# griffithlab/regtools

Hardware: AMD Instinct MI355X
Metric: alignments/sec + junctions/sec, junctions extract, 1/2/4/8 MI355X (higher is better)
Workload: dtype u8/u32 integer; 1 GPU; configs[1]: synthetic 50000000-read 101 bp BAM per GPU, ~15% reads with one N-op, junctions extract -s XS; reads_per_gpu=50000000, seed=1, bgzf_members=169426, compressed_bytes_per_gpu=533101619, inflated_bytes_per_gpu=11060000978

## Files before the change

regtools_amd/csrc/api_internal.h:

```cpp
#pragma once
#include "../../include/regtools_amd.h"

#include <hip/hip_runtime.h>
#include <stdarg.h>
#include <stdio.h>
#include <stdlib.h>
#include <string.h>

#include <algorithm>
#include <atomic>
#include <condition_variable>
#include <charconv>
#include <chrono>
#include <map>
#include <memory>
#include <mutex>
#include <string>
#include <thread>
#include <unordered_map>
#include <vector>

#include "cse_host.h"
#include "host_io.h"
#include "worker_pool.h"
// ... 78 lines not shown
        k.v.erase(k.v.begin() + (long)best);
        return base;
    }
    static void unmap_range(void *base, const std::vector<size_t> &lens, size_t reserved, int dev) {
        static const bool trace = getenv("REGTOOLS_AMD_TRACE") != nullptr;
        size_t at = 0;
        for (size_t n : lens) {
            const hipError_t e = hipMemUnmap((uint8_t *)base + at, n);
            if (e != hipSuccess && trace) fprintf(stderr, "[rgx trace] hipMemUnmap of %zu bytes at +%zu: %s\n", n, at, hipGetErrorString(e));
            if (e != hipSuccess) (void)hipGetLastError();
            at += n;
        }
        KeptRanges &k = kept_ranges();
        std::lock_guard<std::mutex> lock(k.mu);
        k.v.push_back(KeptRange{base, reserved, dev});
    }
    hipError_t map_pieces(size_t bytes, void **out) {
        int dev = 0;
        hipError_t e = hipGetDevice(&dev);
        if (e != hipSuccess) return e;
        hipMemAllocationProp prop = {}; prop.type = hipMemAllocationTypePinned; prop.location.type = hipMemLocationTypeDevice; prop.location.id = dev;
        size_t gran = 0;
        if (hipMemGetAllocationGranularity(&gran, &prop, hipMemAllocationGranularityRecommended) != hipSuccess || !gran) { (void)hipGetLastError();
            gran = (size_t)2 << 20; }
        const size_t total = (bytes + gran - 1) / gran * gran, each = std::max(gran, piece / gran * gran);
        size_t reserved = total;
        void *base = take_range(dev, total, &reserved);
        if (!base) { reserved = total; if ((e = hipMemAddressReserve(&base, total, 0, nullptr, 0)) != hipSuccess) return e; }
        std::vector<size_t> lens;
        size_t done = 0;
        while (done < total) {
            const size_t n = std::min(each, total - done);
            hipMemGenericAllocationHandle_t h;
            if ((e = hipMemCreate(&h, n, &prop, 0)) != hipSuccess) break;
            e = hipMemMap((uint8_t *)base + done, n, 0, h, 0);
            (void)hipMemRelease(h);
            if (e != hipSuccess) break;
            lens.push_back(n);
            done += n;
        }
        if (e == hipSuccess) {
            hipMemAccessDesc ad = {}; ad.location.type = hipMemLocationTypeDevice; ad.location.id = dev; ad.flags = hipMemAccessFlagsProtReadWrite;
            e = hipMemSetAccess(base, total, &ad, 1);
        }
        if (e != hipSuccess) { unmap_range(base, lens, reserved, dev); return e; }
        *out = base; mapped = reserved; range_dev = dev; piece_len.swap(lens);
        return hipSuccess;
    }
    hipError_t ensure(size_t bytes) {
        if (bytes <= cap) return hipSuccess;
        static const bool trace = getenv("REGTOOLS_AMD_TRACE") != nullptr;
        const auto t0 = std::chrono::steady_clock::now();
        release();
        static const bool no_slack = [] { const char *e = getenv("REGTOOLS_AMD_ONE_SHOT"); return e && strcmp(e, "0") != 0; }();
        size_t want = bytes + (no_slack ? 0 : bytes / 8) + 256;
        void *raw = nullptr;
        hipError_t e = hipErrorNotSupported;
        if (piece && want + kFront >= piece) { e = map_pieces(want + kFront, &raw); if (e != hipSuccess) { (void)hipGetLastError(); raw = nullptr;
            mapped = 0; piece_len.clear(); } }
        if (e != hipSuccess) e = hipMalloc(&raw, want + kFront);
        if (e == hipSuccess) { p = (uint8_t *)raw + kFront; cap = want; }
        if (trace) {
            static std::mutex mu; std::lock_guard<std::mutex> lock(mu);
            g_alloc_stats.ms += std::chrono::duration<double, std::milli>(std::chrono::steady_clock::now() - t0).count(); ++g_alloc_stats.calls;
                g_alloc_stats.bytes += want;
        }
        return e;
    }
    void release() {
        if (p && mapped) { (void)hipDeviceSynchronize();
                           unmap_range((uint8_t *)p - kFront, piece_len, mapped, range_dev); }
        else if (p) (void)hipFree((uint8_t *)p - kFront);
        p = nullptr; cap = 0; mapped = 0; piece_len.clear();
    }
    template <class T> T *as() const { return (T *)p; }
    explicit operator Carve() const { return Carve(p, cap); }
};

enum class Buf {
    arena, bad_members, bam, barcode_text, barcodes, cand, cse_assoc, cse_events_all, cse_junction_items, cse_junctions, cse_pairs, cse_variant_hits,
    cse_variants, cse_windows, discover, events, fasta, fasta_tab, gate_done, gate_flags, gtf_tables, hdr_arena, inflate_scratch, members, merge, odd_aux,
    partials, probe_sizes, probe_slots, rank, row_map, rows_out, rows_packed, scalars, seg, seg_chunks, seg_cp, soa, sort, stage, table_dev, tmp, unique,
    count
};

struct RadixSort {
    uint32_t *perm[2], *tmp; uint32_t n; hipStream_t st; uint32_t *key[2] = {nullptr, nullptr};
    int cur = -1;
    const uint32_t *in() const { return cur < 0 ? nullptr : perm[cur]; }
    void passes(const uint32_t *word, uint32_t nbits, int kc) {
        for (uint32_t sh = 0; sh < nbits; sh += 8) {
            const uint32_t bits = std::min<uint32_t>(8, nbits - sh); const int nxt = cur < 0 ? 0 : cur ^ 1;
            if (kc < 0) launch_radix_pass(word, sh, bits, in(), perm[nxt], n, tmp, st);
            else { launch_radix_pass_keyed(word, key[kc], sh, bits, in(), perm[nxt], n, tmp, st); word = key[kc]; kc ^= 1; }
            cur = nxt;
        }
    }
    void by(const uint32_t *word, uint32_t nbits) { passes(word, nbits, -1); }
    void by_keyed(const uint32_t *word, uint32_t nbits) {
        if (cur < 0) return passes(word, nbits, 0);
        launch_gather_u32(n, word, perm[cur], key[0], st);
        passes(key[0], nbits, 1);
    }
    template <class G> void by_gathered(G gather, uint32_t nbits) { gather(in(), key[0]); passes(key[0], nbits, 1); }
    const uint32_t *sorted() const { return perm[cur]; }
    uint32_t *spare() const { return perm[cur ^ 1]; }
    void reset() { cur = -1; }
};

constexpr uint32_t kCcBatch = 4;
struct EdgeList { const uint32_t *a, *b; uint32_t n; };
int components_run(uint32_t n_vertices, const EdgeList *lists, int n_lists, uint32_t *parent, uint32_t *d_flags, hipStream_t st, uint32_t *n_rounds,
                   char *err, size_t errlen);

constexpr int kSideStreams = 2;
struct OverlapKnobs { size_t min_bytes = (size_t)8 << 20; unsigned chunks = 16; uint32_t early_min = 4096; bool early_small = false; };
inline const OverlapKnobs &overlap_knobs() {
    static const OverlapKnobs k = [] {
        OverlapKnobs v;
        if (const char *e = getenv("REGTOOLS_AMD_OVERLAP")) {
            long long a = -1, b = -1, c2 = -1;
            const int n = sscanf(e, "%lld,%lld,%lld", &a, &b, &c2);
            if (n >= 1 && a >= 0) v.min_bytes = (size_t)a;
            if (n >= 2 && b >= 2) v.chunks = (unsigned)std::min<long long>(b, 64);
            if (n >= 3 && c2 >= 1) { v.early_min = (uint32_t)c2; v.early_small = true; }
        }
        return v;
    }();
    return k;
}
struct Turn {
    std::mutex mu; std::condition_variable cv; uint64_t next = 0, serving = 0;
    uint64_t width = 1;
};
struct LinkTurn { Turn wire, chip; };
struct TurnHold {
    Turn *t = nullptr; std::atomic<bool> held{false};
    void take(Turn *x) {
        if (!x || held.load()) return;
        std::unique_lock<std::mutex> lk(x->mu);
        const uint64_t mine = x->next++;
        x->cv.wait(lk, [&] { return mine < x->serving + x->width; });
        t = x; held.store(true);
    }
    void give() { if (held.exchange(false)) { { std::lock_guard<std::mutex> lk(t->mu); ++t->serving; } t->cv.notify_all(); } }
};

struct rgx_ctx {
    int device = 0;
    LinkTurn *link = nullptr;
    TurnHold wire_hold, chip_hold;
    hipStream_t stream = nullptr;
    hipStream_t copy_stream = nullptr, side[kSideStreams] = {};
    bool gate_distrust = false, early_distrust = false;
    bool walk_strict = false;
    bool one_shot = false;
    std::vector<hipEvent_t> chunk_ev;
    uint32_t gate_epoch = 0;
    hipEvent_t ev_ready = nullptr, ev_side[kSideStreams] = {}, ev_packed = nullptr;
    hipEvent_t ev[8] = {};
    uint64_t arena_calibrated_bytes = 0;
    DevBuf *arena_retired = nullptr;
    hipEvent_t ev_trial[2] = {};
    float arena_trial_ms[8] = {}; int arena_trials = 0;
    hipEvent_t ev_launch[2] = {}; bool launch_timed = false;
    DevBuf bufs[(size_t)Buf::count];
    void *pinned = nullptr; size_t pinned_cap = 0;
    std::vector<Member> hm_scratch;
    void *pinned_members = nullptr; size_t pinned_members_cap = 0;
    void *pinned_rows = nullptr; size_t pinned_rows_cap = 0;
    uint64_t last_rows = 0, last_records = 0, last_events = 0, last_bytes = 0; bool last_rows_valid = false;
    struct KPend { hipEvent_t a, b; int slot; };
    std::vector<KPend> kpend; std::vector<hipEvent_t> kfree; double kms[3] = {0, 0, 0};
    uint64_t tables_made = 0;
    std::vector<uint32_t> rank_stage;
    std::string fasta_path;
    rgx::Fasta *fasta = nullptr;
    rgx::Fasta *host_fasta = nullptr; std::string host_fasta_path; uint64_t host_fasta_key[4] = {0, 0, 0, 0};
    DevBuf &buf(Buf b) { return bufs[(size_t)b]; }
};


rgx::Fasta *host_fasta(rgx_ctx *c, const char *path);
void ktime_begin(rgx_ctx *c, int slot);
void ktime_end(rgx_ctx *c);
void ktime_collect(rgx_ctx *c);
hipError_t ensure_upload_streams(rgx_ctx *c);
rgx_junction_table *table_alloc(const BamHeader &h, uint64_t n, bool zero = true, bool pinned = false);
void host_sort_rows(rgx_junction_table *t);
void format_bed12_rows(const rgx_junction_table *t, int only_anchored, uint64_t r0, uint64_t r1, std::string &out);
void *block_take(size_t need, size_t &cap, bool pinned);
void block_give(void *p, size_t cap, bool pinned);
struct TableBox { rgx_junction_table t; void *block; size_t block_cap; bool pinned; };
struct CachedBlock { void *p; size_t cap; bool pinned; };
struct SharedMembers { const std::vector<Member> *members; uint64_t total_inflated; };

struct Prep {
    BamHeader hdr;
    const uint8_t *arena = nullptr;
    ReadSoA soa{};
    EventSoA ev{};
    uint32_t n_rec = 0, n_events = 0, n_range = 0;
    uint64_t n_iterated = 0, total = 0;
    uint32_t framing_sweeps = 0;
    bool stream_ended = false;
    double t_begin = 0;
    struct OddAux { int32_t tid, pos, end; };
    std::vector<OddAux> odd_aux;
    const uint8_t *d_file = nullptr;
};

int prepare_events(rgx_ctx *c, const uint8_t *d_bam_in, const uint8_t *h_bam, size_t bam_len, const uint8_t *bai, size_t bai_len,
                          const rgx_extract_params *p, bool want_read_span, Prep &P, char *err, size_t errlen, const uint32_t *d_true_sizes = nullptr,
                          bool allow_overlap = true, bool region_to_file_end = false, const SharedMembers *shared = nullptr);

constexpr int kGoOn = -1;

struct EventsRun {
    rgx_ctx *c; const uint8_t *d_bam_in; const uint8_t *h_bam; size_t bam_len; const uint8_t *bai; size_t bai_len;
    const rgx_extract_params *p; bool want_read_span; Prep &P; char *err; size_t errlen; const uint32_t *d_true_sizes;
    bool allow_overlap, region_to_file_end; const SharedMembers *shared;
    hipStream_t st = nullptr, copy_q = nullptr;
    double t_begin = 0, t_last = 0; bool trace = false;
    void mark(const char *what) { if (trace) { double t = now_ms(); fprintf(stderr, "[rgx trace] %-28s +%8.3f ms  (at %8.3f)%s\n", what, t - t_last,
        t - t_begin, c->link ? (" clock " + std::to_string(fmod(t, 1e5))).c_str() : ""); t_last = t; } }
    BaiInfo bi; bool bai_ok = false;
    std::vector<uint8_t> index_image;
    std::thread bai_thread;
    const uint8_t *d_bam = nullptr;
    struct Upload {
        std::thread th; std::atomic<uint32_t> recorded{0}; std::atomic<int> err{0};
        std::vector<size_t> end;
        size_t lo = 0, hi = 0, hdr_hi = 0;
        hipStream_t copy_stream = nullptr;
        ~Upload() { if (th.joinable()) th.join(); if (copy_stream) (void)hipStreamSynchronize(copy_stream); }
    } up;
    bool overlap = false, gated = false;
    size_t gate_chunk = 0;
    uint64_t hm_total = 0;
    Scalars *d_sc = nullptr, *h_sc = nullptr;
    template <class T> hipError_t fetch(T &host_member) { return fetch_scalar(d_sc, h_sc, host_member, st); }
    hipError_t complete_upload() {
        if (!h_bam || !(up.lo || (up.hi && up.hi < bam_len))) return hipSuccess;
        if (up.th.joinable()) up.th.join();
        hipError_t e = hipStreamSynchronize(copy_q);
        uint8_t *dst = c->buf(Buf::bam).as<uint8_t>();
        if (e == hipSuccess && up.lo > up.hdr_hi) e = hipMemcpy(dst + up.hdr_hi, h_bam + up.hdr_hi, up.lo - up.hdr_hi, hipMemcpyHostToDevice);
        if (e == hipSuccess && up.hi < bam_len) e = hipMemcpy(dst + up.hi, h_bam + up.hi, bam_len - up.hi, hipMemcpyHostToDevice);
        up.lo = 0; up.hi = bam_len; up.hdr_hi = 0;
        return e;
    }
    uint32_t n_cand = 0;
    uint64_t *cand = nullptr;
    uint32_t *nx[2] = {nullptr, nullptr}, *c_isize = nullptr, *c_reach = nullptr, *c_rank = nullptr, *c_isz2 = nullptr, *c_tmp = nullptr;
    Member *d_members = nullptr; hipMemcpyKind from_members = hipMemcpyDeviceToHost;
    void chain(uint64_t root2) {
        launch_member_link(d_bam, bam_len, cand, n_cand, nx[0], c_isize, c_reach, root2, st);
        int cur = 0;
        for (uint32_t span = 1; span < n_cand; span <<= 1) { launch_member_jump(n_cand, nx[cur], nx[cur ^ 1], c_reach, st); cur ^= 1; }
        launch_member_jump(n_cand, nx[cur], nx[cur ^ 1], c_reach, st);
        launch_scan_u32(c_reach, c_rank, n_cand, &d_sc->n_members, c_tmp, st);
        launch_member_compact(d_bam, bam_len, cand, c_isize, c_reach, c_rank, n_cand, d_members, c_isz2, st);
        if (d_true_sizes) launch_member_fix(d_members, c_isz2, n_cand, &d_sc->n_members, d_true_sizes, st);
        launch_member_upos(d_members, c_isz2, &d_sc->n_members, &d_sc->total_inflated, st);
    }
    bool whole = false, seek = false, chunked = false, geom_chunked_hint = false, empty_stream = false;
    uint64_t seek_voff = 0, cut_lo = 0, cut_hi = UINT64_MAX, total_all = 0, q_upos[3] = {0, 0, 0};
    std::vector<VChunk> chunks;
    uint32_t n_members_all = 0, first_member = 0, stop = 0;
    uint32_t m_lo = 0, m_hi = 0, n_range = 0;
    uint64_t upos_lo = 0, total = 0;
    uint8_t *d_bad = nullptr;
    hipError_t member_at(uint32_t k, Member &m) {
        if (from_members == hipMemcpyHostToHost) { memcpy(&m, d_members + k, sizeof m); return hipSuccess; }
        hipError_t e = hipMemcpyAsync(&m, d_members + k, sizeof m, from_members, st);
        return e == hipSuccess ? hipStreamSynchronize(st) : e;
    }
    hipError_t upos_of(uint32_t k, uint64_t &out_v) {
        if (k >= n_members_all) { out_v = total_all; return hipSuccess; }
        Member m;
        hipError_t e = member_at(k, m);
        out_v = m.upos;
        return e;
    }
    struct EarlyPart { uint32_t members, waves; uint64_t upos; };
    std::vector<EarlyPart> early_parts;
    bool split_B = false; hipEvent_t split_ev = nullptr;
    hipError_t join_B() {
        if (!split_B) return hipSuccess;
        split_B = false;
        return hipStreamWaitEvent(st, split_ev, 0);
    }
    bool spec = false; uint32_t mean_rec = 0;
    BamHeader hdr; int32_t n_ref = 0;
    uint64_t lim = 0, pos0 = 0; bool chain_ended = false;
    ExtractCfg cfg; SegGeom geom; uint32_t seg_bytes = 0;
    std::vector<SegChunk> seg_chunks;
    const uint8_t *arena = nullptr; uint64_t span = 0; uint32_t n_seg = 0, n_rec = 0; bool lite_walk = false;
    uint64_t *seg_start[2] = {nullptr, nullptr}, *seg_exit[2] = {nullptr, nullptr};
    uint32_t *seg_cnt[2] = {nullptr, nullptr}, *seg_base = nullptr;
    uint32_t *seg_iter_e = nullptr, *seg_long_e = nullptr, *seg_long_base_e = nullptr;
    uint16_t *seg_cp = nullptr;
    int cur = 0;
    int frame(uint32_t n_s, uint32_t walk_from, bool &ended) {
        DevBuf &b_tmp = c->buf(Buf::tmp);
        launch_seg_walk(arena, geom, n_s, n_ref, seg_start[cur], seg_exit[cur], seg_cnt[cur], seg_cp, st, walk_from);
        for (int iter = 0;; ++iter) {
            HIP_TRY(hipMemsetAsync(&d_sc->framing, 0xff, sizeof d_sc->framing, st));
            launch_seg_verify(arena, geom, n_s, seg_start[cur], seg_exit[cur], seg_cnt[cur], seg_start[cur ^ 1], seg_exit[cur ^ 1],
                              seg_cnt[cur ^ 1], &d_sc->framing.disagree, seg_cp, st);
            cur ^= 1;
            launch_scan_u32(seg_cnt[cur], seg_base, n_s, &d_sc->n_rec, b_tmp.as<uint32_t>(), st);
            HIP_TRY(fetch(h_sc->n_rec));
            HIP_TRY(fetch(h_sc->framing));
            if (spec && iter == 0) {
                HIP_TRY(fetch(h_sc->inflate));
                HIP_TRY(fetch(h_sc->inflate_early));
            }
            HIP_TRY(hipStreamSynchronize(st));
            if (spec && iter == 0 && (h_sc->inflate.first_bad != 0xffffffffu || h_sc->inflate_early.first_bad != 0xffffffffu)) {
                mark("inflate verdict: not clean, starting over device-resident");
                if (gated) { c->gate_distrust = true; if (trace) fprintf(stderr,
                    "[rgx trace] arrival gate: verdict not clean, this context no longer uses it\n"); }
                HIP_TRY(join_B());
                HIP_TRY(complete_upload());
                HIP_TRY(hipStreamSynchronize(copy_q));
                HIP_TRY(hipStreamSynchronize(st));
                const int rc2 = prepare_events(c, d_bam, nullptr, bam_len, bai, bai_len, p, want_read_span, P, err, errlen, nullptr, false, region_to_file_end);
                P.t_begin = t_begin;
                return rc2;
            }
            ++P.framing_sweeps;
            const Scalars::Framing &fr = h_sc->framing;
            if (fr.chain_end != 0xffffffffu) ended = true;
            if (fr.chain_end != 0xffffffffu && (fr.chain_end < fr.disagree || (fr.disagree == 0xffffffffu && geom.chunks))) {
                launch_seg_truncate(geom, n_s, fr.chain_end, seg_start[cur], seg_exit[cur], seg_cnt[cur], st);
                launch_scan_u32(seg_cnt[cur], seg_base, n_s, &d_sc->n_rec, b_tmp.as<uint32_t>(), st);
                HIP_TRY(fetch(h_sc->n_rec));
                HIP_TRY(hipStreamSynchronize(st));
                break;
            }
            if (fr.disagree == 0xffffffffu) break;
            if (iter > 1 << 20) return fail(err, errlen, RGX_ERR_FORMAT, "regtools_amd: record framing did not converge\n");
        }
        return -1;
    }
    uint32_t sA = 0;
    bool emit_parts_ok = false; uint32_t emit_parts = 0, emit_rows = 0; size_t ev_lay = 0;
    EventSoA ev_e;
    static constexpr size_t kEventRowBytes = 8 * sizeof(uint32_t) + 1;
    EventSoA ev_layout(Carve &w, size_t E) {
        EventSoA v; memset(&v, 0, sizeof v);
        v.tid = w.u32(E); v.start = w.u32(E); v.ilen_cls = w.u32(E); v.ts = w.u32(E); v.te = w.u32(E);
        if (want_read_span) { v.rpos = w.u32(E); v.rend = w.u32(E); }
        if (p->barcodes) v.read = w.u32(E);
        v.strand = w.u8(E);
        return v;
    }
    size_t soa_cap = 0;
    ReadSoA soa;
    uint32_t *ev_base = nullptr, *long_list = nullptr;
    static constexpr size_t kSoaRowBytes = sizeof(uint64_t) + 6 * sizeof(uint32_t) + 1, kSoaRecOffBytes = sizeof(uint64_t);
    int soa_layout(size_t R) {
        DevBuf &b_soa = c->buf(Buf::soa);
        HIP_TRY(b_soa.ensure(R * (kSoaRowBytes + (p->barcodes ? kSoaRecOffBytes : 0)) + 256));
        Carve w(b_soa);
        soa.cig_off = w.u64(R);
        if (p->barcodes) soa.rec_off = w.u64(R);
        soa.tid = w.take<int32_t>(R); soa.pos = w.take<int32_t>(R); soa.flag_nc = w.u32(R);
        soa.n_ev = w.u32(R); ev_base = w.u32(R); long_list = w.u32(R);
        soa.strand = w.u8(R); CARVE_TRY(w, "soa");
        soa_cap = R;
        return kGoOn;
    }
    uint32_t n_events = 0, n_long = 0; uint64_t n_iterated = 0;
    ~EventsRun() {
        if (split_B && split_ev) (void)hipEventSynchronize(split_ev);
        if (bai_thread.joinable()) bai_thread.join();
        if (c->link && !d_bam_in) { c->wire_hold.give(); c->chip_hold.give(); }
    }
    int run();
    int calibrate_arena();
    int stage_upload();
    int stage_members();
    int stage_range_and_inflate();
    int stage_footers_and_header();
    int stage_bounds_and_chains();
    int stage_framing();
    int stage_decode();
    int stage_emit();
};
struct HostRows {
    std::vector<uint32_t> group, start, end, ts, te, count, name_rank, first_seen, last_seen;
    std::vector<uint8_t> strand;
    size_t n = 0;
    const uint32_t *cols = nullptr;
    void append(const HostRows &batch, uint32_t first_window) {
        auto app = [](std::vector<uint32_t> &dst, const std::vector<uint32_t> &src) { dst.insert(dst.end(), src.begin(), src.end()); };
        for (uint32_t g : batch.group) group.push_back(g + first_window);
        app(start, batch.start); app(end, batch.end); app(ts, batch.ts); app(te, batch.te); app(count, batch.count);
        app(name_rank, batch.name_rank); app(first_seen, batch.first_seen); app(last_seen, batch.last_seen);
        strand.insert(strand.end(), batch.strand.begin(), batch.strand.end());
        n += batch.n;
    }
};

struct RowMap { uint32_t *ev_urow = nullptr, *urow_pos = nullptr; };
struct TableSink { const BamHeader *hdr = nullptr; uint32_t min_anchor = 0; rgx_junction_table *table = nullptr; };

int reduce_events(rgx_ctx *c, EventSoA ev, uint32_t n_events, uint32_t group_bits, uint32_t ilen_bits, const uint32_t *rank_of_group_host,
                  uint32_t n_groups, HostRows &R, char *err, size_t errlen, bool view_only = false, RowMap *row_map = nullptr, TableSink *sink = nullptr,
                  bool allow_preagg = true );
int barcode_rows(rgx_ctx *c, const Prep &P, const RowMap &rm, const rgx_extract_params *p, rgx_junction_table *t, char *err, size_t errlen);
void chrom_string_ranks(const BamHeader &hdr, std::vector<uint32_t> &rank_of_tid);
int run_pipeline(rgx_ctx *c, const uint8_t *d_bam_in, const uint8_t *h_bam, size_t bam_len, const uint8_t *bai, size_t bai_len,
                 const rgx_extract_params *p, rgx_junction_table **out, char *err, size_t errlen, const SharedMembers *shared = nullptr);
bool rgx_enable_peer(int a, int b);
int rgx_last_table_pack_async(rgx_ctx *c, const rgx_junction_table *t, void **d_packed, hipEvent_t *done, char *err, size_t errlen);
```

regtools_amd/csrc/api_records.cpp:

```cpp
#include "api_internal.h"

int EventsRun::stage_footers_and_header() {
    DevBuf &b_arena = c->buf(Buf::arena), &b_hdr = c->buf(Buf::hdr_arena), &b_lens = c->buf(Buf::inflate_scratch);
    BamHeader hdr_host;
    mean_rec = 0;
    spec = overlap && !d_true_sizes && !geom_chunked_hint && host_bam_header(h_bam, std::min<size_t>(bam_len, (size_t)8 << 20), hdr_host, nullptr, &mean_rec);
    if (spec) h_sc->inflate = h_sc->inflate_early = InflateStatus{0xffffffffu, 0xffffffffu};
    else {
        HIP_TRY(join_B());
        HIP_TRY(fetch(h_sc->inflate));
        HIP_TRY(fetch(h_sc->inflate_early));
        HIP_TRY(hipStreamSynchronize(st));
    }
    if (!d_true_sizes) {
        auto size_trouble = [](const InflateStatus &s) { return s.first_bad != 0xffffffffu &&
            (s.code == 12u  || s.code == 10u ); };
        bool lies = size_trouble(h_sc->inflate) || size_trouble(h_sc->inflate_early);
        if (!lies && stop < n_members_all) {
            Member ms; uint8_t two[2] = {0, 0};
            HIP_TRY(member_at(stop, ms));
            if (ms.isize == 0 && ms.clen >= 2) {
                if (h_bam && ms.cpos + 2 <= bam_len) memcpy(two, h_bam + ms.cpos, 2);
                else { HIP_TRY(hipMemcpyAsync(two, d_bam + ms.cpos, 2, hipMemcpyDeviceToHost, st)); HIP_TRY(hipStreamSynchronize(st)); }
            }
            lies = !(ms.isize == 0 && two[0] == 3 && two[1] == 0) && ms.isize != 0xffffffffu;
        }
        if (lies) {
            mark("footer mismatch: probing");
            DevBuf &b_slots = c->buf(Buf::probe_slots), &b_sizes = c->buf(Buf::probe_sizes);
            HIP_TRY(b_slots.ensure((size_t)n_members_all * kBgzfMaxBlock + 256));
            HIP_TRY(b_sizes.ensure((size_t)n_members_all * 4 + 64));
            HIP_TRY(b_lens.ensure(inflate_scratch_bytes(std::max<uint32_t>(n_members_all, 64))));
            launch_inflate_probe(d_bam, d_members, n_members_all, b_slots.as<uint8_t>(), b_lens.as<uint32_t>(), b_sizes.as<uint32_t>(), st);
            HIP_TRY(hipStreamSynchronize(st));
            b_slots.release();
            const int rc2 = prepare_events(c, d_bam_in, h_bam, bam_len, bai, bai_len, p, want_read_span, P, err, errlen, b_sizes.as<uint32_t>(), true,
                region_to_file_end);
            P.t_begin = t_begin;
            return rc2;
        }
    }

    if (spec) hdr = hdr_host;
    else {
        const uint32_t h_early = h_sc->inflate_early.first_bad;
        uint32_t n_h = std::min<uint32_t>(n_members_all, 4);
        for (;;) {
            const uint8_t *src; uint64_t have;
            uint32_t bad_h = 0xffffffffu;
            std::vector<Member> hmem(n_h);
            HIP_TRY(hipMemcpyAsync(hmem.data(), d_members, (size_t)n_h * sizeof(Member), from_members, st));
            HIP_TRY(hipStreamSynchronize(st));
            uint32_t used = 0;
            for (; used < n_h; ++used) if (hmem[used].isize == 0 || hmem[used].isize > kBgzfMaxBlock) break;
            if (!used) return fail(err, errlen, RGX_ERR_REGION, "%s", kMsgRegion);
            have = hmem[used - 1].upos + hmem[used - 1].isize;
            if (m_lo == 0 && used <= n_range) src = b_arena.as<uint8_t>();
            else {
                HIP_TRY(b_hdr.ensure(have + 256));
                HIP_TRY(hipMemsetAsync(&d_sc->hdr_inflate.first_bad, 0xff, 4, st));
                launch_inflate(d_bam, d_members, used, b_hdr.as<uint8_t>(), 0, b_lens.as<uint32_t>(), &d_sc->hdr_inflate.first_bad, st);
                src = b_hdr.as<uint8_t>();
            }
            std::vector<uint8_t> hbuf(have);
            HIP_TRY(hipMemcpyAsync(hbuf.data(), src, have, hipMemcpyDeviceToHost, st));
            HIP_TRY(hipMemcpyAsync(h_sc, d_sc, kScalarsHeaderPart, hipMemcpyDeviceToHost, st));
            HIP_TRY(hipStreamSynchronize(st));
            bad_h = (src == b_arena.as<uint8_t>()) ? std::min(h_sc->inflate.first_bad, h_early) : h_sc->hdr_inflate.first_bad;
            if (bad_h != 0xffffffffu && bad_h < used) have = hmem[bad_h].upos;
            uint64_t need = 0;
            int r = parse_bam_header(hbuf.data(), have, hdr, need);
            if (r == 0) {
                uint64_t o = hdr.end, sum = 0; uint32_t cnt = 0;
                while (o + 4 <= have) {
                    uint32_t bl; memcpy(&bl, hbuf.data() + o, 4);
                    if (bl < 32 || bl > (1u << 27) || o + 4 + bl > have) break;
                    sum += 4 + (uint64_t)bl; ++cnt; o += 4 + (uint64_t)bl;
                }
                if (cnt >= 4) mean_rec = (uint32_t)(sum / cnt);
                break;
            }
            if (r == 2 || used < n_h || n_h == n_members_all || (bad_h != 0xffffffffu && bad_h < used))
                return fail(err, errlen, RGX_ERR_REGION, "%s", kMsgRegion);
            n_h = std::min(n_members_all, n_h * 4);
        }
    }
    n_ref = (int32_t)hdr.names.size();
    mark("header (sync: inflate done)");

    return kGoOn;
}

int EventsRun::stage_bounds_and_chains() {
    lim = total;
    if (h_sc->inflate.first_bad != 0xffffffffu) {
        uint64_t u = 0;
        HIP_TRY(upos_of(m_lo + h_sc->inflate.first_bad, u));
        lim = u - upos_lo;
    }
    auto arena_of = [&](uint64_t voff, uint32_t idx, uint64_t upos) -> uint64_t {
        if (idx >= n_members_all || idx < m_lo || idx >= m_hi) return total;
        return std::min<uint64_t>(total, upos - upos_lo + (voff & 0xffff));
    };
    if (cut_lo) pos0 = arena_of(cut_lo, h_sc->q_index[1], q_upos[1]);
    else pos0 = hdr.end;
    chain_ended = false;
    P.stream_ended = empty_stream;
    if (cut_hi != UINT64_MAX) {
        const uint64_t cut_lim = arena_of(cut_hi, h_sc->q_index[2], q_upos[2]);
        const uint32_t mh = h_sc->q_index[2];
        const uint32_t hi_wanted = (mh < n_members_all && (cut_hi & 0xffff)) ? mh + 1 : mh;
        if (!chunked && h_sc->inflate.first_bad != 0xffffffffu && lim < cut_lim) P.stream_ended = true;
        if (!chunked && stop < std::min(hi_wanted, n_members_all)) P.stream_ended = true;
        lim = std::min(lim, cut_lim);
    } else if (h_sc->inflate.first_bad != 0xffffffffu) P.stream_ended = true;
    if (pos0 > lim) pos0 = lim;
    if (empty_stream) lim = pos0;

    memset(&cfg, 0, sizeof cfg);
    cfg.n_ref = n_ref; cfg.strandness = p->strandness; cfg.tag0 = (uint8_t)p->strand_tag[0]; cfg.tag1 = (uint8_t)p->strand_tag[1];
    if ((p->strandness == 0 || p->barcodes) && !want_read_span) { cfg.abort_out = &d_sc->abort_row; HIP_TRY(hipMemsetAsync(&d_sc->abort_row, 0xff, 4, st)); }
    if (p->barcodes && !want_read_span) { cfg.bc0 = (uint8_t)p->barcode_tag[0]; cfg.bc1 = (uint8_t)p->barcode_tag[1]; }
    if (p->strandness == 0 && want_read_span) { cfg.odd_count = &d_sc->odd_aux; HIP_TRY(hipMemsetAsync(&d_sc->odd_aux, 0, 4, st)); }
    P.odd_aux.clear();
    cfg.min_anchor = p->min_anchor; cfg.min_intron = p->min_intron; cfg.max_intron = p->max_intron;
    cfg.region_tid = -2; cfg.long_threshold = 16;
    if (!whole) {
        int32_t tid, beg, end;
        if (!parse_region(hdr, p->region, tid, beg, end) || tid >= bi.n_ref || end < beg)
            return fail(err, errlen, RGX_ERR_REGION, "%s", kMsgRegion);
        cfg.region_tid = tid; cfg.region_beg = beg; cfg.region_end = end;
    }

    if (p->fasta_path) {
        if (!c->fasta || c->fasta_path != p->fasta_path) {
            delete c->fasta; c->fasta = new Fasta(); c->fasta_path.clear();
            if (!c->fasta->load(p->fasta_path)) { delete c->fasta; c->fasta = nullptr; return fail(err, errlen, RGX_ERR_FASTA,
                "Unable to open FASTA file.\n\n"); }
            DevBuf &bf = c->buf(Buf::fasta);
            HIP_TRY(bf.ensure(c->fasta->size + 256));
            HIP_TRY(hipMemcpy(bf.p, c->fasta->data, c->fasta->size, hipMemcpyHostToDevice));
            c->fasta_path = p->fasta_path;
        }
        std::vector<FaContig> tab((size_t)std::max(n_ref, 1));
        memset(tab.data(), 0, tab.size() * sizeof(FaContig));
        for (int32_t t = 0; t < n_ref; ++t)
            for (const Fasta::Seq &s : c->fasta->seqs)
                if (s.name == hdr.names[(size_t)t]) {
                    const bool sane = s.offset >= 0 && s.len >= 0 && s.line_blen > 0 && s.line_len >= s.line_blen &&
                                      (s.len == 0 ||
                                          (uint64_t)s.offset + (uint64_t)((s.len - 1) / s.line_blen) * (uint64_t)s.line_len +
                                                  (uint64_t)((s.len - 1) % s.line_blen) < (uint64_t)c->fasta->size);
                    if (!sane) continue;
                    tab[(size_t)t].offset = s.offset; tab[(size_t)t].len = s.len; tab[(size_t)t].line_blen = s.line_blen;
                        tab[(size_t)t].line_len = s.line_len; tab[(size_t)t].present = 1;
                }
        DevBuf &bt = c->buf(Buf::fasta_tab);
        HIP_TRY(bt.ensure(tab.size() * sizeof(FaContig) + 64));
        HIP_TRY(hipMemcpy(bt.p, tab.data(), tab.size() * sizeof(FaContig), hipMemcpyHostToDevice));
        cfg.fa_data = c->buf(Buf::fasta).as<uint8_t>(); cfg.fa_tab = bt.as<FaContig>(); cfg.fa_missing = &d_sc->fa_missing;
    }

    memset(&geom, 0, sizeof geom);
    const int env_seg = decode_knobs().seg_bytes;
    seg_bytes = env_seg == (int)kSegBytes || env_seg == (int)kSegBytesLong ? (uint32_t)env_seg : (mean_rec >= kLongRecordBytes ? kSegBytesLong : kSegBytes);
    geom.seg_bytes = seg_bytes;
    if (chunked && chunks.empty()) lim = pos0;
    if (chunked && !chunks.empty() && !empty_stream) {
        std::vector<Member> rm(n_range);
        std::vector<uint8_t> bad(n_range, 0);
        if (n_range) {
            HIP_TRY(hipMemcpyAsync(rm.data(), d_members + m_lo, (size_t)n_range * sizeof(Member), from_members, st));
            HIP_TRY(hipMemcpyAsync(bad.data(), d_bad, n_range, hipMemcpyDeviceToHost, st));
            HIP_TRY(hipStreamSynchronize(st));
        }
        for (uint32_t k = 0; k < n_range; ++k) if (rm[k].isize == 0 || rm[k].isize > kBgzfMaxBlock) bad[k] = 1;
        std::vector<uint32_t> next_bad((size_t)n_range + 1, n_range);
        for (uint32_t k = n_range; k-- > 0;) next_bad[k] = bad[k] ? k : next_bad[k + 1];
        auto usize = [&](uint32_t k) { return rm[k].isize <= kBgzfMaxBlock ? rm[k].isize : 0u; };
        auto lower = [&](uint64_t cfile) {
            uint32_t lo_ = 0, hi_ = n_range;
            while (lo_ < hi_) { const uint32_t mid = lo_ + (hi_ - lo_) / 2; if (rm[mid].cpos - 18 < cfile) lo_ = mid + 1; else hi_ = mid; }
            return lo_;
        };
        uint32_t seg_total = 0;
        for (const VChunk &ch : chunks) {
            const uint32_t k = lower(ch.u >> 16);
            if (k >= n_range || rm[k].cpos - 18 != (ch.u >> 16)) break;
            SegChunk sc; memset(&sc, 0, sizeof sc);
            sc.a = rm[k].upos - upos_lo + std::min<uint64_t>(ch.u & 0xffff, usize(k));
            const uint32_t kv = lower(ch.v >> 16);
            if (kv >= n_range) sc.b = total;
            else sc.b = rm[kv].upos - upos_lo + (rm[kv].cpos - 18 == (ch.v >> 16) ? std::min<uint64_t>(ch.v & 0xffff, usize(kv)) : 0);
            if (sc.b <= sc.a) sc.b = sc.a + 1;
            const uint32_t nb = next_bad[k];
            sc.dlim = nb < n_range ? rm[nb].upos - upos_lo : total;
            sc.seg_base = seg_total;
            const uint64_t ns = (sc.b - sc.a + seg_bytes - 1) / seg_bytes;
            if (seg_total + ns > 0x7fffffffull) return fail(err, errlen, RGX_ERR_FORMAT, "regtools_amd: region too large\n");
            seg_total += (uint32_t)ns;
            seg_chunks.push_back(sc);
        }
        if (seg_chunks.empty()) lim = pos0;
        else {
            DevBuf &b_ch = c->buf(Buf::seg_chunks);
            HIP_TRY(b_ch.ensure(seg_chunks.size() * sizeof(SegChunk) + 64));
            HIP_TRY(hipMemcpyAsync(b_ch.p, seg_chunks.data(), seg_chunks.size() * sizeof(SegChunk), hipMemcpyHostToDevice, st));
            geom.chunks = b_ch.as<SegChunk>(); geom.n_chunks = (uint32_t)seg_chunks.size();
        }
        mark("chunk table");
    }

    return kGoOn;
}

int EventsRun::stage_framing() {
    arena = c->buf(Buf::arena).as<uint8_t>();
    span = lim - pos0;
    n_seg = (uint32_t)((span + seg_bytes - 1) / seg_bytes);
    geom.pos0 = pos0; geom.lim = lim; geom.data_end = lim; geom.seg_bytes = seg_bytes;
    const int env_lite = 1;
    lite_walk = env_lite && !c->walk_strict;
    geom.lite_walk = lite_walk ? 1u : 0u;
    if (geom.chunks) {
        span = 0;
        for (const SegChunk &sc : seg_chunks) span += sc.b - sc.a;
        const SegChunk &lastc = seg_chunks.back();
        n_seg = lastc.seg_base + (uint32_t)((lastc.b - lastc.a + seg_bytes - 1) / seg_bytes);
        geom.data_end = total;
    }
    n_rec = 0;
    DevBuf &b_seg = c->buf(Buf::seg), &b_tmp = c->buf(Buf::tmp);
    HIP_TRY(hipEventRecord(c->ev[2], st));
    sA = 0;
    emit_parts_ok = false; emit_parts = 0; emit_rows = 0; ev_lay = 0;
    memset(&ev_e, 0, sizeof ev_e);
    soa_cap = 0;
    memset(&soa, 0, sizeof soa);
    ev_base = nullptr; long_list = nullptr;
    if (n_seg) {
        const size_t per = (size_t)n_seg;
        HIP_TRY(b_seg.ensure(per * (8 + 8 + 4) * 2 + per * 4 + per * 12 + 64));
        HIP_TRY(c->buf(Buf::seg_cp).ensure(per * kSegCpSlots * 2 + 64));
        seg_cp = c->buf(Buf::seg_cp).as<uint16_t>();
        Carve q(b_seg);
        for (int k = 0; k < 2; ++k) { seg_start[k] = q.u64(per); seg_exit[k] = q.u64(per); }
        for (int k = 0; k < 2; ++k) seg_cnt[k] = q.u32(per);
        seg_base = q.u32(per);
        seg_iter_e = q.u32(per); seg_long_e = q.u32(per); seg_long_base_e = q.u32(per); CARVE_TRY(q, "seg");
        HIP_TRY(b_tmp.ensure(scan_tmp_words(n_seg) * 4 + 64));
        bool early = split_B && spec && !geom.chunks && seg_bytes == kSegBytes && cut_hi == UINT64_MAX && !empty_stream && lim == total;
        const bool env_early_emit = true;
        const bool small_ok = overlap_knobs().early_small;
        uint32_t waves_done = 0;
        for (size_t j = 0; early && j < early_parts.size(); ++j) {
            const EarlyPart &ep = early_parts[j];
            if (ep.upos <= pos0 + 2 * (uint64_t)kBgzfMaxBlock) continue;
            uint32_t sJ = (uint32_t)std::min<uint64_t>(n_seg, (ep.upos - kBgzfMaxBlock - pos0) / seg_bytes);
            if (small_ok ? (sJ < sA + 2 || n_seg - sJ < 1) : (sJ < sA + 1024 || n_seg - sJ < 64)) continue;
            HIP_TRY(hipMemsetAsync(&d_sc->wait_timed_out, 0, 4, st));
            for (size_t i = 0; i <= j; ++i) {
                const uint32_t w_end = early_parts[i].waves, w_beg = i ? early_parts[i - 1].waves : 0u;
                if (w_end > waves_done) { launch_wait_done(c->buf(Buf::gate_done).as<uint32_t>() + i, w_end - w_beg, &d_sc->wait_timed_out, st); waves_done = w_end; }
            }
            HIP_TRY(fetch(h_sc->wait_timed_out));
            if (trace) fprintf(stderr, "[rgx trace] early tail: part %zu: members < %u, segments [%u, %u) of %u\n", j, ep.members, sA, sJ, n_seg);
            bool ended_J = false;
            const uint32_t sweeps0 = P.framing_sweeps;
            const int rcJ = frame(sJ, sA, ended_J);
            if (rcJ != -1) return rcJ;
            const uint32_t n_rec_J = h_sc->n_rec;
            uint64_t exit_J = 0;
            HIP_TRY(hipMemcpyAsync(&h_sc->exit_staging, seg_exit[cur] + (sJ - 1), 8, hipMemcpyDeviceToHost, st));
            HIP_TRY(hipStreamSynchronize(st));
            exit_J = h_sc->exit_staging;
            const bool reaches_J = exit_J > ep.upos;
            if (reaches_J && trace) fprintf(stderr,
                "[rgx trace] early tail: a record of the prefix ends at %llu, behind the inflated part (%llu): one pass\n", (unsigned long long)exit_J,
                (unsigned long long)ep.upos);
            const bool slow_J = P.framing_sweeps - sweeps0 > 2;
            P.framing_sweeps = sweeps0;
            const uint64_t span_J = (uint64_t)sJ * seg_bytes;
            if (h_sc->wait_timed_out) { c->early_distrust = true; if (trace) fprintf(stderr,
                "[rgx trace] early tail: a wait for a part's waves timed out, this context no longer uses it\n"); }
            if (h_sc->wait_timed_out || ended_J || slow_J || reaches_J || !n_rec_J || span_J / n_rec_J > kSparseRecordBytes ||
                (sA && n_rec_J > soa_cap)) { early = false; sA = 0; emit_parts_ok = false; emit_parts = 0; emit_rows = 0; break; }
            if (!sA) {
                { const int rc = soa_layout((size_t)((double)n_rec_J * ((double)n_seg / sJ) * 1.125) + 65536); if (rc != kGoOn) return rc; }
                cfg.insane_out = nullptr;
                if (lite_walk) { cfg.insane_out = &d_sc->insane; HIP_TRY(hipMemsetAsync(&d_sc->insane, 0, 4, st)); h_sc->insane = 0; }
            }
            launch_decode_seg(arena, geom, sJ, seg_start[cur], seg_base, seg_cnt[cur], cfg, soa, seg_iter_e, seg_long_e, seg_cp, true, st, sA);
            if (!sA) {
                DevBuf &b_ev0 = c->buf(Buf::events);
                ev_lay = b_ev0.cap > 256 ? (b_ev0.cap - 256) / kEventRowBytes : 0;
                emit_parts_ok = env_early_emit && ev_lay >= 4096;
                if (emit_parts_ok) { HIP_TRY(b_tmp.ensure(scan_tmp_words((uint32_t)std::min<size_t>(soa_cap, 0xffffffffu)) * 4 + 64));
                    Carve w(b_ev0); ev_e = ev_layout(w, ev_lay); CARVE_TRY(w, "events"); }
            }
            if (emit_parts_ok && emit_parts < kGateParts - 1) {
                launch_scan_u32(soa.n_ev + emit_rows, ev_base + emit_rows, n_rec_J - emit_rows, d_sc->part_events + emit_parts, b_tmp.as<uint32_t>(), st);
                launch_emit_short(arena, n_rec_J, cfg, soa, ev_base, ev_e, st, emit_rows, d_sc->part_events, emit_parts, (uint32_t)std::min<size_t>(ev_lay,
                    0xffffffffu));
                emit_rows = n_rec_J; ++emit_parts;
            }
            sA = sJ;
            mark("early tail: part framed and decoded");
        }
        HIP_TRY(join_B());
        const int rcF = frame(n_seg, sA, chain_ended);
        if (rcF != -1) return rcF;
        n_rec = h_sc->n_rec;
    } else HIP_TRY(join_B());
    if (spec && !n_seg) {
        HIP_TRY(fetch(h_sc->inflate));
        HIP_TRY(fetch(h_sc->inflate_early));
        HIP_TRY(hipStreamSynchronize(st));
        if (h_sc->inflate.first_bad != 0xffffffffu || h_sc->inflate_early.first_bad != 0xffffffffu) {
            HIP_TRY(complete_upload());
            HIP_TRY(hipStreamSynchronize(copy_q));
            const int rc2 = prepare_events(c, d_bam, nullptr, bam_len, bai, bai_len, p, want_read_span, P, err, errlen, nullptr, false, region_to_file_end);
            P.t_begin = t_begin;
            return rc2;
        }
    }
    if (chain_ended) P.stream_ended = true;
    if (chain_ended && geom.chunks && m_hi < n_members_all && !region_to_file_end) {
        mark("region: chain ended, re-reading to the end of the file");
        if (overlap) { HIP_TRY(complete_upload()); HIP_TRY(hipStreamSynchronize(copy_q)); }
        const int rc2 = prepare_events(c, d_bam, nullptr, bam_len, bai, bai_len, p, want_read_span, P, err, errlen, d_true_sizes, false, true);
        P.t_begin = t_begin;
        return rc2;
    }
    HIP_TRY(hipEventRecord(c->ev[3], st));
    mark("framing (sync)");

    return kGoOn;
}

int EventsRun::stage_decode() {
    DevBuf &b_tmp = c->buf(Buf::tmp);
    n_events = 0; n_long = 0;
    n_iterated = 0;
    if (n_rec) {
        const size_t R = n_rec;
        uint32_t s_from = sA;
        if (sA && (R > soa_cap || chain_ended)) s_from = 0;
        if (!s_from) { const int rc = soa_layout(R); if (rc != kGoOn) return rc; emit_parts_ok = false; }
        HIP_TRY(b_tmp.ensure(scan_tmp_words(n_rec) * 4 + 64));
        uint32_t *seg_iter = sA ? seg_iter_e : seg_cnt[cur ^ 1], *seg_long = sA ? seg_long_e : (uint32_t *)seg_start[cur ^ 1], *seg_long_base = sA ?
            seg_long_base_e : (uint32_t *)seg_exit[cur ^ 1];
        if (geom.chunks) {
            cfg.stop_out = &d_sc->stop_rule.index; cfg.stop_index = 0xffffffffu;
            HIP_TRY(hipMemsetAsync(&d_sc->stop_rule.index, 0xff, 4, st));
            HIP_TRY(hipMemsetAsync(&d_sc->stop_rule.last_pass, 0, 4, st));
        }
        if (!s_from) {
            cfg.insane_out = nullptr;
            if (lite_walk) { cfg.insane_out = &d_sc->insane; HIP_TRY(hipMemsetAsync(&d_sc->insane, 0, 4, st)); h_sc->insane = 0; }
        }
        for (int pass = 0; pass < 2; ++pass) {
            launch_decode_seg(arena, geom, n_seg, seg_start[cur], seg_base, seg_cnt[cur], cfg, soa, seg_iter, seg_long, seg_cp,
                              span / n_rec <= kSparseRecordBytes, st, s_from);
            if (emit_parts_ok && s_from) {
                launch_scan_u32(soa.n_ev + emit_rows, ev_base + emit_rows, n_rec - emit_rows, d_sc->part_events + emit_parts, b_tmp.as<uint32_t>(), st);
                launch_emit_short(arena, n_rec, cfg, soa, ev_base, ev_e, st, emit_rows, d_sc->part_events, emit_parts,
                    (uint32_t)std::min<size_t>(ev_lay, 0xffffffffu));
                HIP_TRY(fetch(h_sc->part_events));
            } else launch_scan_u32(soa.n_ev, ev_base, n_rec, &d_sc->counts.n_events, b_tmp.as<uint32_t>(), st);
            launch_scan_u32(seg_iter, seg_iter, n_seg, &d_sc->counts.n_iterated, b_tmp.as<uint32_t>(), st);
            launch_scan_u32(seg_long, seg_long_base, n_seg, &d_sc->counts.n_long, b_tmp.as<uint32_t>(), st);
            HIP_TRY(fetch(h_sc->counts));
            if (cfg.stop_out) HIP_TRY(fetch(h_sc->stop_rule));
            if (cfg.insane_out) HIP_TRY(fetch(h_sc->insane));
            if (cfg.abort_out) HIP_TRY(fetch(h_sc->abort_row));
            if (cfg.odd_count) HIP_TRY(fetch(h_sc->odd_aux));
            HIP_TRY(hipStreamSynchronize(st));
            if (cfg.insane_out && h_sc->insane) {
                mark("decode: a record fails bam_read1's test, starting over with the full walk");
                if (overlap) { HIP_TRY(complete_upload()); HIP_TRY(hipStreamSynchronize(copy_q)); }
                c->walk_strict = true;
                const int rc2 = prepare_events(c, d_bam, nullptr, bam_len, bai, bai_len, p, want_read_span, P, err, errlen, d_true_sizes, false,
                    region_to_file_end);
                c->walk_strict = false;
                P.t_begin = t_begin;
                return rc2;
            }
            if (pass || !cfg.stop_out || h_sc->stop_rule.index == 0xffffffffu || h_sc->stop_rule.last_pass <= h_sc->stop_rule.index + 1) break;
            cfg.stop_index = h_sc->stop_rule.index;
        }
        if (cfg.abort_out && h_sc->abort_row != 0xffffffffu && h_sc->abort_row < (cfg.stop_out ? cfg.stop_index : 0xffffffffu))
            return fail(err, errlen, RGX_ERR_ABORT,
                "regtools_amd: record %u has an auxiliary field of unknown type in front of its strand or barcode tag: the reference abort()s here\n",
                h_sc->abort_row);
        n_events = h_sc->counts.n_events; n_long = h_sc->counts.n_long;
        if (emit_parts_ok && s_from) {
            uint64_t tot = 0;
            for (uint32_t k = 0; k <= emit_parts && k < kGateParts; ++k) tot += h_sc->part_events[k];
            if (tot > ev_lay || tot > 0xffffffffull || n_long) {
                emit_parts_ok = false;
                launch_scan_u32(soa.n_ev, ev_base, n_rec, &d_sc->counts.n_events, b_tmp.as<uint32_t>(), st);
                HIP_TRY(fetch(h_sc->counts.n_events));
                HIP_TRY(hipStreamSynchronize(st));
                n_events = h_sc->counts.n_events;
            } else n_events = (uint32_t)tot;
        }
        n_iterated = h_sc->counts.n_iterated;
        if (cfg.odd_count && h_sc->odd_aux) {
            const uint32_t cap = h_sc->odd_aux;
            DevBuf &b_odd = c->buf(Buf::odd_aux);
            HIP_TRY(b_odd.ensure((size_t)cap * 12 + 16));
            HIP_TRY(hipMemsetAsync(&d_sc->odd_aux, 0, 4, st));
            launch_collect_odd_aux(arena, soa, n_rec, cap, &d_sc->odd_aux, b_odd.as<int32_t>(), st);
            HIP_TRY(fetch(h_sc->odd_aux));
            HIP_TRY(hipStreamSynchronize(st));
            const uint32_t n_odd = std::min(h_sc->odd_aux, cap);
            std::vector<int32_t> rows((size_t)n_odd * 3);
            if (n_odd) { HIP_TRY(hipMemcpyAsync(rows.data(), b_odd.p, (size_t)n_odd * 12, hipMemcpyDeviceToHost, st)); HIP_TRY(hipStreamSynchronize(st)); }
            for (uint32_t k = 0; k < n_odd; ++k) P.odd_aux.push_back(Prep::OddAux{rows[3 * (size_t)k], rows[3 * (size_t)k + 1], rows[3 * (size_t)k + 2]});
        }
        if (geom.chunks && p->n_shards > 1 && h_sc->stop_rule.index != 0xffffffffu) P.stream_ended = true;
        if (n_long) launch_long_fill(n_seg, seg_base, seg_cnt[cur], seg_long_base, cfg, soa, long_list, st);
    }
    HIP_TRY(hipEventRecord(c->ev[4], st));
    mark("decode+count (sync)");

    return kGoOn;
}

int EventsRun::stage_emit() {
    DevBuf &b_ev = c->buf(Buf::events);
    EventSoA ev; memset(&ev, 0, sizeof ev);
    if (n_events) {
        const size_t E = n_events;
        if (emit_parts_ok && n_rec) ev = ev_e;
        else {
            HIP_TRY(b_ev.ensure(E * kEventRowBytes + 256));
            Carve w(b_ev); ev = ev_layout(w, E); CARVE_TRY(w, "events");
            launch_emit_short(arena, n_rec, cfg, soa, ev_base, ev, st);
            launch_emit_long(arena, long_list, n_long, cfg, soa, ev_base, ev, st);
        }
        if (cfg.fa_data) {
            HIP_TRY(fetch(h_sc->fa_missing));
            HIP_TRY(hipStreamSynchronize(st));
            if (h_sc->fa_missing) return fail(err, errlen, RGX_ERR_FASTA, "Unable to extract FASTA sequence for position %s\n\n",
                hdr.names[(size_t)(h_sc->fa_missing - 1)].c_str());
        }
    }
    HIP_TRY(hipEventRecord(c->ev[5], st));

    P.hdr = hdr; P.arena = arena; P.soa = soa; P.ev = ev; P.n_rec = n_rec; P.n_events = n_events; P.n_range = n_range;
    P.n_iterated = n_iterated; P.total = total; P.t_begin = t_begin;
    return RGX_OK;
}

int prepare_events(rgx_ctx *c, const uint8_t *d_bam_in, const uint8_t *h_bam, size_t bam_len, const uint8_t *bai, size_t bai_len,
                          const rgx_extract_params *p, bool want_read_span, Prep &P, char *err, size_t errlen, const uint32_t *d_true_sizes,
                          bool allow_overlap, bool region_to_file_end, const SharedMembers *shared) {
    EventsRun r{c, d_bam_in, h_bam, bam_len, bai, bai_len, p, want_read_span, P, err, errlen, d_true_sizes, allow_overlap, region_to_file_end, shared};
    return r.run();
}
```

regtools_amd/csrc/bam_core.h:

```cpp
#pragma once
#include "common.h"

namespace rgx {

struct RecHead {
    int32_t  block_len;
    int32_t  tid, pos;
    uint32_t l_qname, n_cigar, flag;
    int32_t  l_qseq;
    int32_t  mtid;
    int64_t  aux_off;
};

RGX_HD void rec_head(const uint8_t *a, RecHead &h) {
    h.block_len = (int32_t)ld32(a);
    h.tid = (int32_t)ld32(a + 4); h.pos = (int32_t)ld32(a + 8);
    uint32_t x2 = ld32(a + 12), x3 = ld32(a + 16);
    h.l_qname = x2 & 0xff; h.n_cigar = x3 & 0xffff; h.flag = x3 >> 16;
    h.l_qseq = (int32_t)ld32(a + 20);
    h.mtid = (int32_t)ld32(a + 24);
    h.aux_off = (int64_t)h.l_qname + 4 * (int64_t)h.n_cigar + (((int64_t)h.l_qseq + 1) >> 1) + h.l_qseq;
}

RGX_HD bool rec_sane(const RecHead &h) {
    int64_t l_data = (int64_t)h.block_len - 32;
    if (l_data < 0 || h.l_qseq < 0 || h.l_qname < 1) return false;
    return h.aux_off <= l_data;
}

RGX_HD bool rec_plausible(const uint8_t *arena, uint64_t o, uint64_t lim, int32_t n_ref) {
    if (o + 36 > lim) return false;
    RecHead h; rec_head(arena + o, h);
    if (!rec_sane(h)) return false;
    if (h.block_len > (1 << 27)) return false;
    if (h.tid < -1 || h.tid >= n_ref || h.mtid < -1 || h.mtid >= n_ref) return false;
    if (h.pos < -1 || h.pos > (1 << 29)) return false;
    uint64_t q_end = o + 36 + h.l_qname - 1;
    if (q_end < lim && arena[q_end] != 0) return false;
    return true;
}

RGX_HD char strand_from_flag(uint32_t flag, int strandness) {
    int rev = (flag >> 4) & 1, mrev = (flag >> 5) & 1, r1 = (flag >> 6) & 1, r2 = (flag >> 7) & 1;
    int nb = (strandness - 1) == 0 ? 1 : 0;
    int f = nb ^ r1 ^ rev, s = nb ^ r2 ^ mrev;
    return f != s ? '?' : (f ? '+' : '-');
}

RGX_HD char strand_from_tag(const uint8_t *aux, const uint8_t *end, uint8_t t0, uint8_t t1, bool *unknown = nullptr) {
    const uint8_t *s = aux;
    while (s + 3 <= end) {
        bool hit = s[0] == t0 && s[1] == t1;
        s += 2;
        if (hit) return (s[0] == 'A' && s + 2 <= end && s[1] != 0) ? (char)s[1] : '?';
        uint8_t t = *s++;
        uint32_t sz;
        switch (t) {
            case 'A': case 'c': case 'C': sz = 1; break;
            case 's': case 'S': sz = 2; break;
            case 'i': case 'I': case 'f': sz = 4; break;
            case 'd': sz = 8; break;
            case 'Z': case 'H': { while (s < end && *s) ++s; sz = 1; break; }
            case 'B': {
                if (s + 5 > end) return '?';
                uint8_t st = *s++; uint32_t n = (uint32_t)s[0] | (uint32_t)s[1] << 8 | (uint32_t)s[2] << 16 | (uint32_t)s[3] << 24; s += 4;
                uint32_t es = (st == 'c' || st == 'C' || st == 'A') ? 1 : (st == 's' || st == 'S') ? 2 : (st == 'i' || st == 'I' || st == 'f') ? 4 : (st == 'd') ? 8 : 0;
                if ((uint64_t)es * n > (uint64_t)(end - s)) return '?';
                sz = es * n; break;
            }
            default: if (unknown) *unknown = true; return '?';
        }
        s += sz;
    }
    return '?';
}

RGX_HD int aux_find_string(const uint8_t *aux, const uint8_t *end, uint8_t t0, uint8_t t1, uint32_t *val, uint32_t *len) {
    const uint8_t *s = aux;
    while (s + 3 <= end) {
        const bool hit = s[0] == t0 && s[1] == t1;
        s += 2;
        const uint8_t t = *s++;
        if (hit) {
            if (t != 'Z' && t != 'H') return -1;
            const uint8_t *e = s;
            while (e < end && *e) ++e;
            *val = (uint32_t)(s - aux); *len = (uint32_t)(e - s);
            return 1;
        }
        uint32_t sz;
        switch (t) {
            case 'A': case 'c': case 'C': sz = 1; break;
            case 's': case 'S': sz = 2; break;
            case 'i': case 'I': case 'f': sz = 4; break;
            case 'd': sz = 8; break;
            case 'Z': case 'H': { while (s < end && *s) ++s; sz = 1; break; }
            case 'B': {
                if (s + 5 > end) return 0;
                uint8_t st = *s++; uint32_t n = (uint32_t)s[0] | (uint32_t)s[1] << 8 | (uint32_t)s[2] << 16 | (uint32_t)s[3] << 24; s += 4;
                uint32_t es = (st == 'c' || st == 'C' || st == 'A') ? 1 : (st == 's' || st == 'S') ? 2 : (st == 'i' || st == 'I' || st == 'f') ? 4 : (st == 'd') ? 8 : 0;
                if ((uint64_t)es * n > (uint64_t)(end - s)) return 0;
                sz = es * n; break;
            }
            default: return 0;
        }
        s += sz;
    }
    return 0;
}
RGX_HD void barcode_hash(const uint8_t *s, uint32_t len, uint32_t *lo, uint32_t *hi) {
    uint32_t a = 0x811c9dc5u ^ len, b = 0x9747b28cu + len * 0x85ebca6bu;
    for (uint32_t i = 0; i < len; ++i) {
        a = (a ^ s[i]) * 0x01000193u;
        b = (b + s[i]) * 0xcc9e2d51u; b = (b << 15 | b >> 17) * 0x1b873593u;
    }
    a ^= a >> 16; a *= 0x7feb352du; a ^= a >> 15;
    b ^= b >> 13; b *= 0xc2b2ae35u; b ^= b >> 16;
    *lo = a; *hi = b;
}

struct FaContig { int64_t offset, len; int32_t line_blen, line_len; int32_t present; int32_t pad; };

RGX_HD int fa_fetch2(const uint8_t *fa, const FaContig &c, uint32_t beg1, uint32_t end1, uint8_t *b) {
    int64_t beg = beg1, end = end1;
    if (beg > 0) --beg;
    if (beg >= c.len) beg = c.len;
    if (end >= c.len) end = c.len;
    if (beg > end) beg = end;
    int n = 0;
    if (c.line_blen <= 0) return 0;
    for (int64_t p = beg; p < end && n < 2; ++p) b[n++] = fa[c.offset + p / c.line_blen * c.line_len + p % c.line_blen];
    return n;
}
RGX_HD uint8_t base_comp(uint8_t c) { return c == 'A' ? 'T' : c == 'C' ? 'G' : c == 'G' ? 'C' : c == 'T' ? 'A' : 'N'; }

RGX_HD char strand_from_motif(const uint8_t *fa, const FaContig &c, uint32_t start, uint32_t end, char carried) {
    uint8_t s1[2], s2[2];
    const int l1 = fa_fetch2(fa, c, start + 1u, start + 2u, s1);
    const int l2 = fa_fetch2(fa, c, end + 1u - 2u, end + 1u - 1u, s2);
    if (l1 != 2 || l2 != 2) return '?';
    uint8_t d0, d1, a0, a1;
    if (carried == '-') { d0 = base_comp(s2[1]); d1 = base_comp(s2[0]); a0 = base_comp(s1[1]); a1 = base_comp(s1[0]); }
    else { d0 = s1[0]; d1 = s1[1]; a0 = s2[0]; a1 = s2[1]; }
    const uint32_t m = (uint32_t)d0 << 24 | (uint32_t)d1 << 16 | (uint32_t)a0 << 8 | a1;
    if (m == 0x47544147u  || m == 0x47434147u  || m == 0x41544143u ) return '+';
    if (m == 0x43544143u  || m == 0x43544743u  || m == 0x47544154u ) return '-';
    return '?';
}

RGX_HD uint32_t strand_class(char c) { return c == '+' ? 0u : c == '-' ? 1u : 2u; }

RGX_HD uint32_t cig_ref_len(uint32_t c) {
    uint32_t op = c & 0xf;
    return ((0x3C1A7u >> (op << 1)) & 2u) ? (c >> 4) : 0u;
}
RGX_HD bool cig_is_N(uint32_t c) { return (c & 0xf) == 3; }
RGX_HD bool cig_is_breaker(uint32_t c) { uint32_t op = c & 0xf; return op == 3 || op == 2 || op == 8 || op == 1 || op == 4; }
RGX_HD bool cig_advances_junction_state(uint32_t c) {
    uint32_t op = c & 0xf; return op == 0 || op == 7 || op == 2 || op == 8 || op == 3;
}

RGX_HD int32_t rec_endpos(const uint8_t *cig, uint32_t n_cigar, uint32_t flag, int32_t pos) {
    if (!(flag & 4) && n_cigar > 0) {
        int32_t l = 0;
        for (uint32_t k = 0; k < n_cigar; ++k) l += (int32_t)cig_ref_len(ld32(cig + 4 * (size_t)k));
        return pos + l;
    }
    return pos + 1;
}

template <class Emit>
RGX_HD void cigar_walk(int32_t pos, const uint8_t *cig, uint32_t n_cigar, Emit &&emit) {
    uint32_t start = (uint32_t)pos, ts = (uint32_t)pos, end = 0, te = 0;
    bool started = false;
    for (uint32_t i = 0; i < n_cigar; ++i) {
        uint32_t c = ld32(cig + 4 * (size_t)i), op = c & 0xf, len = c >> 4;
        if (op == 3) {
            if (!started) { end = start + len; te = end; started = true; }
            else { emit(start, end, ts, te); ts = end; start = te; end = start + len; te = end; }
        } else if (op == 0 || op == 7) {
            if (!started) start += len; else te += len;
        } else if (op == 2 || op == 8) {
            if (!started) { start += len; ts = start; }
            else { emit(start, end, ts, te); start = te + len; ts = start; }
            started = false;
        } else if (op == 1 || op == 4) {
            if (!started) ts = start;
            else { emit(start, end, ts, te); start = te; ts = start; }
            started = false;
        }
    }
    if (started) emit(start, end, ts, te);
}

RGX_HD bool intron_ok(uint32_t start, uint32_t end, uint32_t min_intron, uint32_t max_intron) {
    uint32_t l = end - start;
    return !(l < min_intron || l > max_intron);
}

}
```

regtools_amd/csrc/kernels.h:

```cpp
#pragma once
#include <hip/hip_runtime.h>

#include "common.h"
#include "bam_core.h"

namespace rgx {

constexpr uint32_t kSegBytes = 16384;
constexpr uint32_t kSparseRecordBytes = 2048;
constexpr uint32_t kSegCpSlots = 64;
constexpr uint64_t kChainEnd = ~0ull;
constexpr uint64_t kChainUnknown = ~0ull - 1;

size_t inflate_scratch_bytes(uint32_t n_members);
hipError_t pending_launch_error();
struct InflateGate {
    const uint32_t *flags = nullptr;
    uint32_t epoch = 0;
    uint32_t n_chunks = 0;
    uint64_t lo = 0, chunk_bytes = 1;
    uint32_t *done = nullptr;
    uint32_t part_start[7] = {0xffffffffu, 0xffffffffu, 0xffffffffu, 0xffffffffu, 0xffffffffu, 0xffffffffu, 0xffffffffu};
};
constexpr uint32_t kGateParts = 8;
constexpr uint32_t kInflateSortGroup = 1024;
void launch_wait_done(const uint32_t *done, uint32_t expected, uint32_t *timed_out, hipStream_t stream);
constexpr uint32_t kStatusEarly = 76;
void launch_inflate(const uint8_t *comp, const Member *members, uint32_t n_members, uint8_t *arena, uint64_t upos_bias, uint32_t *len_scratch,
                    uint32_t *status , hipStream_t stream, uint32_t ignore_below = 0 ,
                    uint32_t index_bias = 0 ,
                    bool piece = false ,
                    int form = 0 ,
                    uint8_t *bad_flags = nullptr ,
                    int plan = 1 ,
                    bool check_layout = false ,
                    InflateGate gate = InflateGate() );
bool inflate_takes_coop(uint32_t n_members);
void launch_gate_set(uint32_t *flag, uint32_t epoch, hipStream_t stream);
inline int inflate_plan_for(uint64_t compressed_bytes, uint64_t inflated_bytes) {
    return compressed_bytes * 32 > inflated_bytes ? 1 : 0;
}

constexpr uint32_t kMagicTile = 4096;
void launch_magic_count(const uint8_t *bam, uint64_t len, uint32_t n_tiles, uint32_t *tile_cnt, hipStream_t stream);
void launch_magic_fill(const uint8_t *bam, uint64_t len, uint32_t n_tiles, const uint32_t *tile_base, uint64_t *cand, hipStream_t stream);
void launch_member_link(const uint8_t *bam, uint64_t len, const uint64_t *cand, uint32_t n, uint32_t *next, uint32_t *isize,
                        uint32_t *reach, uint64_t root2 , hipStream_t stream);
void launch_member_jump(uint32_t n, const uint32_t *next_in, uint32_t *next_out, uint32_t *reach, hipStream_t stream);
void launch_member_compact(const uint8_t *bam, uint64_t len, const uint64_t *cand, const uint32_t *isize, const uint32_t *reach, const uint32_t *rank,
                           uint32_t n, Member *members, uint32_t *isize_compact, hipStream_t stream);
void launch_member_upos(Member *members, const uint32_t *isize_compact, const uint32_t *n_members , uint64_t *total, hipStream_t stream);
void launch_member_query(const Member *members, const uint32_t *n_members , const uint64_t *q_coff, uint32_t n_q, uint32_t *q_index,
                         uint64_t *q_upos, hipStream_t stream);
void launch_inflate_probe(const uint8_t *comp, const Member *members, uint32_t n_members, uint8_t *slots, uint32_t *len_scratch, uint32_t *sizes,
                          hipStream_t stream);
void launch_member_fix(Member *members, uint32_t *isize_compact, uint32_t max_members, const uint32_t *n_members , const uint32_t *fix,
                       hipStream_t stream);
void launch_member_stop(const Member *members, uint32_t max_members, const uint32_t *n_members , const uint32_t *from , uint32_t *stop,
                        hipStream_t stream);

struct SegChunk { uint64_t a, b, dlim; uint32_t seg_base, pad; };
struct DecodeKnobs { bool wave_form = false; int seg_bytes = 0; };
const DecodeKnobs &decode_knobs();
struct SegGeom {
    uint64_t pos0, lim;
    uint64_t data_end;
    const SegChunk *chunks; uint32_t n_chunks;
    uint32_t seg_bytes;
    uint32_t lite_walk;
};
constexpr uint32_t kSegBytesLong = 131072;
constexpr uint32_t kLongRecordBytes = 2048;
void launch_seg_walk(const uint8_t *arena, SegGeom g, uint32_t n_seg, int32_t n_ref,
                     uint64_t *seg_start, uint64_t *seg_exit, uint32_t *seg_cnt, uint16_t *seg_cp , hipStream_t stream,
                     uint32_t s_begin = 0 );
void launch_seg_verify(const uint8_t *arena, SegGeom g, uint32_t n_seg,
                       const uint64_t *seg_start_in, const uint64_t *seg_exit_in, const uint32_t *seg_cnt_in,
                       uint64_t *seg_start_out, uint64_t *seg_exit_out, uint32_t *seg_cnt_out,
                       uint32_t *status , uint16_t *seg_cp, hipStream_t stream);
void launch_seg_truncate(SegGeom g, uint32_t n_seg, uint32_t last, uint64_t *seg_start, uint64_t *seg_exit, uint32_t *seg_cnt, hipStream_t stream);

struct ReadSoA {
    int32_t  *tid, *pos;
    uint32_t *flag_nc;
    uint64_t *cig_off;
    uint8_t  *strand;
    uint32_t *n_ev;
    uint64_t *rec_off;
};
struct ExtractCfg {
    int32_t  n_ref;
    int32_t  strandness;
    uint8_t  tag0, tag1;
    uint32_t min_anchor, min_intron, max_intron;
    int32_t  region_tid;
    int32_t  region_beg, region_end;
    uint32_t long_threshold;
    const uint8_t *fa_data;
    const struct FaContig *fa_tab;
    uint32_t *fa_missing;
    uint32_t *stop_out;
    uint32_t stop_index;
    uint32_t *insane_out;
    uint32_t *abort_out;
    uint8_t  bc0, bc1;
    uint32_t *odd_count;
};
void launch_collect_odd_aux(const uint8_t *arena, ReadSoA soa, uint32_t n_rec, uint32_t cap, uint32_t *count, int32_t *out, hipStream_t stream);

void launch_decode_seg(const uint8_t *arena, SegGeom g, uint32_t n_seg, const uint64_t *seg_start, const uint32_t *seg_base,
                       const uint32_t *seg_cnt, ExtractCfg cfg, ReadSoA soa, uint32_t *seg_iter, uint32_t *seg_long, const uint16_t *seg_cp,
                       bool staged , hipStream_t stream,
                       uint32_t s_begin = 0 );
void launch_long_fill(uint32_t n_seg, const uint32_t *seg_base, const uint32_t *seg_cnt, const uint32_t *seg_long_base, ExtractCfg cfg, ReadSoA soa,
                      uint32_t *long_list, hipStream_t stream);

struct EventSoA {
    uint32_t *tid, *start, *ilen_cls;
    uint32_t *ts, *te;
    uint32_t *rpos, *rend;
    uint8_t  *strand;
    uint32_t *read;
};
void launch_emit_short(const uint8_t *arena, uint32_t n_rec, ExtractCfg cfg, ReadSoA soa, const uint32_t *ev_base,
                       EventSoA ev, hipStream_t stream, uint32_t row_begin = 0 ,
                       const uint32_t *part_totals = nullptr, uint32_t n_parts = 0 ,
                       uint32_t slot_cap = 0xffffffffu );
void launch_emit_long(const uint8_t *arena, const uint32_t *long_list, uint32_t n_long,
                      ExtractCfg cfg, ReadSoA soa, const uint32_t *ev_base, EventSoA ev, hipStream_t stream);

size_t scan_tmp_words(uint32_t n);
void launch_scan_u32(const uint32_t *in, uint32_t *out, uint32_t n, uint32_t *total, uint32_t *tmp, hipStream_t stream);

size_t radix_tmp_words(uint32_t n);
void launch_radix_pass(const uint32_t *word, uint32_t shift, uint32_t bits, const uint32_t *perm_in, uint32_t *perm_out,
                       uint32_t n, uint32_t *tmp, hipStream_t stream);
void launch_radix_pass_keyed(const uint32_t *key_in, uint32_t *key_out, uint32_t shift, uint32_t bits, const uint32_t *perm_in, uint32_t *perm_out,
                             uint32_t n, uint32_t *tmp, hipStream_t stream);

struct UniqueSoA {
    uint32_t *tid, *start, *end, *ts_min, *te_max, *count, *first_seen, *last_seen, *name_rank;
    uint8_t  *strand;
};
struct PartialSoA { uint32_t *tid, *start, *ilen_cls, *ts, *te, *count, *first, *last; };
void launch_preagg(EventSoA ev, uint32_t n, PartialSoA p, uint32_t *p_total , hipStream_t stream);
void launch_reduce_partials(PartialSoA p, const uint32_t *perm, const uint32_t *head, const uint32_t *seg_excl, uint32_t n, UniqueSoA u, hipStream_t stream);
void launch_reduce_finish_partials(const uint8_t *ev_strand, uint32_t n_unique, UniqueSoA u, uint32_t *first_flag , hipStream_t stream);
void launch_heads(EventSoA ev, const uint32_t *perm, uint32_t n, uint32_t *head, hipStream_t stream);
void launch_reduce(EventSoA ev, const uint32_t *perm, const uint32_t *head, const uint32_t *seg_excl, uint32_t n, UniqueSoA u,
                   uint32_t *head_pos, hipStream_t stream);
void launch_reduce_finish(EventSoA ev, const uint32_t *perm, uint32_t n, uint32_t n_unique, const uint32_t *head_pos, UniqueSoA u,
                          uint32_t *first_flag, hipStream_t stream);
void launch_name_rank(uint32_t n_unique, const uint32_t *flag_scan, UniqueSoA u, hipStream_t stream);
void launch_gather_u32(uint32_t n, const uint32_t *table, const uint32_t *idx, uint32_t *out, hipStream_t stream);
void launch_fill_u32(uint32_t *p, uint32_t v, size_t n, hipStream_t stream);
void launch_rows_out(UniqueSoA u, const uint32_t *order, uint32_t n, uint32_t *out, hipStream_t stream);
RGX_HD size_t table_block_rows(uint64_t n) { return ((size_t)n + 1 + 15) & ~(size_t)15; }
RGX_HD size_t table_block_bytes(uint64_t n) { return table_block_rows(n) * (8 * 3 + 4 * 6 + 3); }
void launch_rows_table(UniqueSoA u, const uint32_t *order, uint32_t n, uint32_t min_anchor, uint8_t *out, hipStream_t stream);


struct BarcodeEv { uint64_t *off; uint32_t *len, *h_lo, *h_hi, *row; };
void launch_event_urow(const uint32_t *sorted, const uint32_t *head, const uint32_t *seg_excl, uint32_t n, uint32_t *ev_urow, hipStream_t stream);
void launch_inverse_perm(const uint32_t *perm, uint32_t n, uint32_t *inv, hipStream_t stream);
void launch_bc_event_keys(const uint8_t *arena, uint32_t n_events, const uint32_t *ev_read, const uint64_t *rec_off, const uint32_t *ev_urow,
                          const uint32_t *urow_pos, uint8_t t0, uint8_t t1, BarcodeEv b, uint32_t *flags, hipStream_t stream);
void launch_bc_heads(const uint8_t *arena, BarcodeEv b, const uint32_t *perm, uint32_t n, uint32_t *head, uint32_t *flags, hipStream_t stream);
void launch_bc_pairs(BarcodeEv b, const uint32_t *perm, const uint32_t *head, const uint32_t *seg_excl, uint32_t n, uint32_t *pair_row,
                     uint32_t *pair_first, uint32_t *pair_pos, uint64_t *pair_off, uint32_t *pair_len, hipStream_t stream);
void launch_bc_counts(uint32_t n_pairs, uint32_t n, const uint32_t *pair_pos, uint32_t *pair_count, hipStream_t stream);
void launch_bc_gather(const uint8_t *arena, uint32_t n_pairs, const uint64_t *pair_off, const uint32_t *pair_len, const uint32_t *str_begin,
                      uint8_t *text, hipStream_t stream);

struct GtfView;
struct VariantOpts;
}
#include "cse_core.h"
namespace rgx {
void launch_variant_scan(bool fill, GtfView g, uint32_t n, const int32_t *chrom, const uint32_t *pos0, VariantOpts o, uint32_t *count, const uint32_t *base,
                         uint32_t *ces, uint32_t *cee, uint32_t *hit_tx, uint32_t *hit_ad, unsigned long long *visits ,
                         hipStream_t stream, uint32_t *last_score = nullptr );
void launch_junction_scan(bool fill, GtfView g, uint32_t n, const int32_t *chrom, const uint32_t *js, const uint32_t *je, const uint8_t *strand, uint32_t *count,
                          const uint32_t *base, uint32_t *flags, uint32_t *item_kind, uint32_t *item_a, uint32_t *item_b, unsigned long long *visits,
                          uint32_t *visit_each , hipStream_t stream);
void launch_max_span(EventSoA ev, uint32_t n, uint32_t *out , hipStream_t stream);
constexpr uint32_t kWinSlices = 4;
void launch_window_pairs(bool fill, EventSoA ev, uint32_t n_events, uint32_t n_win, const int32_t *w_tid, const int32_t *w_beg, const int32_t *w_end,
                         const uint32_t *max_span, uint32_t *w_lo, uint32_t *w_hi ,
                         uint32_t *count, const uint32_t *base, uint32_t *pair_ev, uint32_t *pair_win, hipStream_t stream);
void launch_assoc_pairs(bool fill, uint32_t n_win, const int32_t *w_chrom, const uint32_t *w_ces, const uint32_t *w_cee, const uint32_t *chrom_off,
                        const uint32_t *j_start, const uint32_t *j_end, uint32_t *count, const uint32_t *base, uint32_t *pair_j, uint32_t *pair_win, hipStream_t stream);
void launch_pair_gather(EventSoA ev, const uint32_t *pair_ev, const uint32_t *pair_win, uint32_t n, EventSoA out, hipStream_t stream);

struct MergeSoA { uint32_t *tid, *start, *end, *ts, *te, *count, *cls, *first, *shard; uint32_t *strand; };
struct MergeUnique { uint32_t *tid, *start, *end, *ts, *te, *count, *first, *last_shard, *strand; };
void launch_merge_unpack(const uint32_t *rows, uint32_t stride_rows, uint32_t n_parts, const uint32_t *part_rows, const uint32_t *part_base, MergeSoA m, hipStream_t st);
void launch_cols_to_packed(const uint32_t *cols , uint32_t n, uint32_t *out, hipStream_t st);
void launch_merge_heads(MergeSoA m, const uint32_t *sorted, uint32_t n, uint32_t *head, hipStream_t st);
void launch_merge_reduce(MergeSoA m, const uint32_t *sorted, const uint32_t *head, const uint32_t *seg_excl, uint32_t n, MergeUnique u , hipStream_t st);
void launch_merge_rank(const uint32_t *by_first, uint32_t n, uint32_t *name_rank, hipStream_t st);
void launch_merge_pack(MergeUnique u, const uint32_t *order, const uint32_t *name_rank, uint32_t n, uint32_t *out, hipStream_t st);
void launch_merge_table(MergeUnique u, const uint32_t *order, const uint32_t *name_rank, uint32_t n, uint32_t min_anchor, uint8_t *out, hipStream_t st);

constexpr uint32_t kCohortBlockLog2 = 22, kCohortBlockRows = 1u << kCohortBlockLog2, kCohortColumns = 7;
struct CohortSorted { uint32_t *tid, *start, *end, *ts, *te, *count, *ss; };
struct CohortRows { uint32_t *ts, *te, *keep, *kept_nnz; unsigned long long *total; };
struct CohortImage { unsigned long long *total, *row_begin; uint32_t *tid, *start, *end, *ts, *te, *n_with, *col_sample, *val_count; uint8_t *strand; };
void launch_cohort_append(const uint32_t *src, uint32_t n, size_t stride, uint32_t strand_col, const uint32_t *tid_map, uint32_t n_map, uint32_t min_anchor,
                          bool only_anchored, uint32_t sample, uint32_t *fill, uint32_t cap, uint32_t *const *blocks, hipStream_t st);
void launch_cohort_key(uint32_t *const *blocks, const uint32_t *perm, uint32_t n, uint32_t which, uint32_t *out, hipStream_t st);
void launch_cohort_gather(uint32_t *const *blocks, const uint32_t *perm, uint32_t n, CohortSorted s, uint32_t *head, hipStream_t st);
void launch_cohort_row_start(const uint32_t *head, const uint32_t *seg_excl, uint32_t n, uint32_t *row_start , hipStream_t st);
void launch_cohort_reduce(CohortSorted s, const uint32_t *row_start, uint32_t n, uint32_t n_rows, uint32_t min_samples, uint64_t min_total, CohortRows r,
                          hipStream_t st);
void launch_cohort_out(CohortSorted s, const uint32_t *head, const uint32_t *seg_excl, const uint32_t *row_start, CohortRows r, const uint32_t *out_row,
                       const uint32_t *nnz_excl, uint32_t n, uint32_t n_rows, uint32_t n_nnz_kept, CohortImage o, hipStream_t st);

void launch_cluster_class(const uint8_t *strand, uint32_t n, uint32_t *cls , hipStream_t st);
void launch_cluster_edges(const uint32_t *perm, const uint32_t *tid, const uint32_t *cls, const uint32_t *site, uint32_t n, uint32_t *ea, uint32_t *eb,
                          hipStream_t st);
void launch_cc_init(uint32_t *parent, uint32_t n, hipStream_t st);
void launch_cc_hook(uint32_t *parent, const uint32_t *a, const uint32_t *b, uint32_t n_edges, uint32_t n_vertices, uint32_t *flag, hipStream_t st);
void launch_cc_jump(uint32_t *parent, uint32_t n, uint32_t *flag, hipStream_t st);
void launch_cluster_tally(const uint32_t *label, const unsigned long long *total, uint32_t n, uint32_t *cnt, unsigned long long *tot, hipStream_t st);
void launch_cluster_roots(const uint32_t *label, const uint32_t *cnt, const unsigned long long *tot, uint32_t n, uint32_t min_rows, uint64_t min_total,
                          uint32_t *is_root, uint32_t *keep, hipStream_t st);
void launch_cluster_assign(const uint32_t *label, const uint32_t *keep, const uint32_t *cid_excl, const uint32_t *cnt, const unsigned long long *tot,
                           uint32_t n, uint32_t n_clusters, uint32_t *cluster, uint32_t *sort_key, uint32_t *cl_count, unsigned long long *cl_total,
                           hipStream_t st);
void launch_cluster_widen(const uint32_t *in, uint32_t n, const uint32_t *last, unsigned long long *out , hipStream_t st);
void launch_cluster_row_len(const uint32_t *cluster, const unsigned long long *row_begin, const uint32_t *val, uint32_t n, bool wave_per_row, uint32_t *len,
                            hipStream_t st);
void launch_cluster_expand(const uint32_t *cluster, const unsigned long long *row_begin, const uint32_t *col, const uint32_t *val, const uint32_t *ent_off,
                           uint32_t n, bool wave_per_row, uint32_t *e_cluster, uint32_t *e_sample, uint32_t *e_count, hipStream_t st);
void launch_cluster_cs_heads(const uint32_t *perm, const uint32_t *e_cluster, const uint32_t *e_sample, uint32_t n, uint32_t *head, hipStream_t st);
void launch_cluster_cs_sum(const uint32_t *perm, const uint32_t *e_cluster, const uint32_t *e_sample, const uint32_t *e_count, const uint32_t *seg_start,
                           uint32_t n, uint32_t n_seg, uint32_t *seg_cluster, uint32_t *cs_sample, unsigned long long *cs_total, hipStream_t st);
void launch_cluster_cs_begin(const uint32_t *seg_cluster, uint32_t n_seg, uint32_t n_clusters, unsigned long long *cs_begin , hipStream_t st);
void launch_refine_eligible(const uint32_t *start, const uint32_t *end, uint32_t n, uint32_t max_intron, uint32_t *alive, hipStream_t st);
void launch_refine_compact(const uint32_t *order, uint32_t k, const uint32_t *alive, uint32_t *pos, uint32_t *out, uint32_t *n_live, uint32_t *tmp,
                           hipStream_t st);
void launch_refine_edges(const uint32_t *perm, const uint32_t *n_live, const uint32_t *tid, const uint32_t *cls, const uint32_t *site, uint32_t cap,
                         uint32_t *ea, uint32_t *eb, hipStream_t st);
void launch_refine_tally(const uint32_t *label, const unsigned long long *total, const uint32_t *alive, uint32_t n, uint32_t *cnt,
                         unsigned long long *tot, hipStream_t st);
void launch_refine_mark(const uint32_t *label, const unsigned long long *total, const unsigned long long *tot, uint32_t n, uint64_t min_reads,
                        uint32_t ratio_num, uint32_t ratio_den, uint32_t *alive, hipStream_t st);
void launch_refine_roots(const uint32_t *label, const uint32_t *cnt, const unsigned long long *tot, const uint32_t *alive, uint32_t n, uint32_t min_rows,
                         uint64_t min_total, uint32_t *is_root, uint32_t *keep, hipStream_t st);

struct PhenoIn { const uint32_t *cluster; const unsigned long long *row_begin; const uint32_t *col_sample, *val_count;
                 const unsigned long long *cs_begin; const uint32_t *cs_sample; const unsigned long long *cs_total; };
void launch_pheno_row_stats(PhenoIn in, uint32_t n, uint32_t n_samples, uint32_t na_num, uint32_t na_den, double min_sd, uint32_t *n_na, double *mean,
                            double *sd, uint32_t *keep, uint32_t *drop_na, hipStream_t st);
void launch_pheno_scatter(const uint32_t *keep, const uint32_t *pos, const uint32_t *n_na, const double *mean, const double *sd, uint32_t n,
                          uint32_t *o_row, uint32_t *o_n_na, double *o_mean, double *o_sd, hipStream_t st);
void launch_pheno_z(PhenoIn in, const uint32_t *o_row, const double *o_mean, const double *o_sd, uint32_t n_kept, uint32_t n_samples, uint32_t *z_lo,
                    uint32_t *z_hi, uint32_t *e_sample, hipStream_t st);
void launch_pheno_tie_heads(const uint32_t *perm, const uint32_t *z_lo, const uint32_t *z_hi, uint32_t n, uint32_t n_kept, uint32_t *head,
                            hipStream_t st);
void launch_pheno_rank(const uint32_t *perm, const uint32_t *head, const uint32_t *seg_excl, const uint32_t *run_start, uint32_t n, uint32_t n_kept,
                       uint32_t *rank2, hipStream_t st);

void launch_pca_gram(const uint32_t *rank2, const double *T, uint64_t K, uint32_t S, double *part, double *col_part, uint32_t *bad, hipStream_t st);
void launch_pca_reduce(const double *part, const double *col_part, uint64_t K, uint32_t S, double *gram, double *col_sum, hipStream_t st);

}
```

regtools_amd/csrc/kernels.hip:

```cpp
#include "kernels.h"

#include <mutex>
#include <type_traits>

#include "bam_core.h"
#include "inflate_core.h"
#include "inflate_coop.h"
#include "inflate_ring.h"
#include "inflate_wave.h"

namespace rgx {

__device__ __forceinline__ uint32_t lane_id() { return threadIdx.x & 63u; }
__device__ __forceinline__ uint64_t lanemask_lt() { return (1ull << lane_id()) - 1ull; }

__device__ __forceinline__ uint32_t wave_incl_scan(uint32_t v) {
#pragma unroll
    for (int d = 1; d < 64; d <<= 1) {
        uint32_t t = __shfl_up(v, d, 64);
        if ((int)lane_id() >= d) v += t;
    }
    return v;
}

// ... 325 lines not shown
        if (have) status[m] = run && st == INF_OK ? out_len : 0xffffffffu;
        return;
    }
    const bool run = have && mb.isize <= kBgzfMaxBlock;
    typedef typename std::conditional<WIN == 1, BitReaderWin, BitReader>::type BR;
    int st = inflate_coop<BR>(comp + mb.cpos, mb.clen, run ? arena + (mb.upos - upos_bias) : C.wave_base, run ? mb.isize : 0, &out_len, T, C, run, pairs);
    if (have) {
        if (!run) st = mb.isize == 0xffffffffu ? INF_IN_OVERRUN : INF_OUT_OVERFLOW;
        else if (st == INF_OK && out_len != mb.isize) st = INF_SIZE_MISMATCH;
        if (st != INF_OK) {
            const uint32_t mi = m + index_bias;
            if (bad) bad[mi] = 1;
            uint32_t *sl = mi >= ignore_below ? status : status + kStatusEarly;
            uint32_t prev = atomicMin(&sl[0], mi);
            if (mi < prev) sl[1] = (uint32_t)st;
        }
    }
    if (PIECE) gate_wave_done(gate, lane);
}

static size_t inflate_scratch_words(uint32_t n_members) { return (size_t)((n_members + 63) / 64) * 64 * kScratchWordsPerLane; }
size_t inflate_scratch_bytes(uint32_t n_members) { return (inflate_scratch_words(n_members) + ((size_t)n_members + 63) / 64 * 64 + kSortGroup) * 4; }

struct DevWave {
    uint32_t lane;
    template <class F> __device__ __forceinline__ void lanes(F f) const { f(lane); }
    __device__ __forceinline__ void sync() const {
        __builtin_amdgcn_fence(__ATOMIC_RELEASE, "workgroup");
        __builtin_amdgcn_s_barrier();
        __builtin_amdgcn_fence(__ATOMIC_ACQUIRE, "workgroup");
    }
};
static_assert(sizeof(WaveShared) <= 80 * 1024, "two wave-per-member workgroups per CU");

__global__ __launch_bounds__(64) void k_inflate_wave(const uint8_t *__restrict__ comp, const Member *__restrict__ members, uint32_t n_members, uint8_t *arena,
                                                     uint64_t upos_bias, uint32_t *status, uint32_t ignore_below, uint32_t index_bias, uint8_t *bad) {
    extern __shared__ __attribute__((aligned(16))) uint32_t lds[];
    WaveShared &S = *reinterpret_cast<WaveShared *>(lds);
    const uint32_t m = blockIdx.x;
    if (m >= n_members) return;
    const Member mb = members[m];
    DevWave W{threadIdx.x};
    int st;
    uint32_t out_len = 0;
    if (mb.isize > kBgzfMaxBlock) st = mb.isize == 0xffffffffu ? INF_IN_OVERRUN : INF_OUT_OVERFLOW;
    else {
        st = inflate_wave(W, S, comp + mb.cpos, mb.clen, arena + (mb.upos - upos_bias), mb.isize, &out_len);
        if (st == INF_OK && out_len != mb.isize) st = INF_SIZE_MISMATCH;
    }
    if (st != INF_OK && threadIdx.x == 0) {
        const uint32_t mi = m + index_bias;
        if (bad) bad[mi] = 1;
        uint32_t *slot = mi >= ignore_below ? status : status + kStatusEarly;
        uint32_t prev = atomicMin(&slot[0], mi);
        if (mi < prev) slot[1] = (uint32_t)st;
    }
}

constexpr uint32_t kWaveFormMaxMembers = 2048;
constexpr int kDefaultLaneForm = 4;
constexpr int kDefaultWindow = 1;
static int inflate_form_env() {
    static const int f = [] {
        const char *e = getenv("REGTOOLS_AMD_INFLATE");
        return !e ? 0 : !strcmp(e, "lane") ? 1 : !strcmp(e, "wave") ? 2 : !strcmp(e, "ring") ? 3 : !strcmp(e, "coop") ? 4 : 0;
    }();
    return f;
}
static thread_local hipError_t tl_launch_error = hipSuccess;
hipError_t pending_launch_error() {
    hipError_t e = tl_launch_error; tl_launch_error = hipSuccess;
    const hipError_t last = hipGetLastError();
    return e != hipSuccess ? e : last;
}
static void inflate_attrs() {
    static std::mutex mu;
    static bool done_dev[64] = {};
    static hipError_t err_dev[64] = {};
    int dev = 0;
    if (hipGetDevice(&dev) != hipSuccess || dev < 0 || dev >= 64) dev = 0;
    std::lock_guard<std::mutex> lk(mu);
    bool &done = done_dev[dev];
    if (done) { if (err_dev[dev] != hipSuccess) tl_launch_error = err_dev[dev]; return; }
    hipError_t first = hipSuccess;
    auto set = [&](const void *fn, uint32_t bytes) { const hipError_t e = hipFuncSetAttribute(fn, hipFuncAttributeMaxDynamicSharedMemorySize, (int)bytes); if (e != hipSuccess && first == hipSuccess) first = e; };
    set((const void *)k_inflate<false, false>, kInflateLdsBytes);
    set((const void *)k_inflate<false, true>, kInflateLdsBytes);
    set((const void *)k_inflate<true>, kInflateLdsBytes);
    set((const void *)k_inflate_coop<false, false, 0>, kInflateLdsBytes);
    set((const void *)k_inflate<false, false, 4>, kInflateLdsBytes);
    set((const void *)k_inflate<false, true, 4>, kInflateLdsBytes);
    set((const void *)k_inflate_coop<false, true, 0>, kInflateLdsBytes);
    set((const void *)k_inflate_coop<false, false, 1>, kInflateLdsBytes);
    set((const void *)k_inflate_coop<false, true, 1>, kInflateLdsBytes);
    set((const void *)k_inflate_coop<true>, kInflateLdsBytes);
    set((const void *)k_inflate_wave, (uint32_t)sizeof(WaveShared));
    set((const void *)k_inflate_ring<false>, kRingLdsBytes);
    set((const void *)k_inflate_ring<true>, kRingLdsBytes);
    err_dev[dev] = first; done = true;
    if (first != hipSuccess) tl_launch_error = first;
}
__global__ void k_gate_set(uint32_t *flag, uint32_t epoch) { __hip_atomic_store(flag, epoch, __ATOMIC_RELAXED, __HIP_MEMORY_SCOPE_SYSTEM); }
void launch_gate_set(uint32_t *flag, uint32_t epoch, hipStream_t stream) { hipLaunchKernelGGL(k_gate_set, dim3(1), dim3(1), 0, stream, flag, epoch); }
bool inflate_takes_coop(uint32_t n_members) {
    const int f = inflate_form_env();
    return f ? f == 4 : n_members > kWaveFormMaxMembers && kDefaultLaneForm == 4;
}
void launch_inflate(const uint8_t *comp, const Member *members, uint32_t n_members, uint8_t *arena, uint64_t upos_bias, uint32_t *len_scratch,
                    uint32_t *status, hipStream_t stream, uint32_t ignore_below, uint32_t index_bias, bool piece, int form, uint8_t *bad, int plan, bool check_layout, InflateGate gate) {
    if (!n_members) return;
    inflate_attrs();
    const uint32_t two = (plan & 1) ? 7u : 4u;
    if (!form) form = inflate_form_env();
    if (!form) form = n_members <= kWaveFormMaxMembers ? 2 : (plan & 2) ? 1 : kDefaultLaneForm;
    const uint32_t blocks = (n_members + 63) / 64;
    switch (form) {
    case 2:
        hipLaunchKernelGGL(k_inflate_wave, dim3(n_members), dim3(64), (uint32_t)sizeof(WaveShared), stream, comp, members, n_members, arena, upos_bias, status, ignore_below, index_bias, bad);
        break;
    case 3:
        hipLaunchKernelGGL(k_inflate_ring<false>, dim3(blocks), dim3(64), kRingLdsBytes, stream, comp, members, n_members, arena, upos_bias, len_scratch, status, ignore_below, index_bias, bad);
        break;
    case 4: {
        const bool sort = (plan & 1) != 0;
        const int win = kDefaultWindow;
        uint32_t *perm = sort ? len_scratch + inflate_scratch_words(n_members) : nullptr;
        if (perm) hipLaunchKernelGGL(k_member_sort, dim3((n_members + kSortGroup - 1) / kSortGroup), dim3(256), 0, stream, members, n_members, perm);
        uint32_t *veto = check_layout ? len_scratch + inflate_scratch_words(n_members) + ((size_t)n_members + 63) / 64 * 64 + kSortGroup - 1 : nullptr;
        if (check_layout) {
            (void)hipMemsetAsync(veto, 0, 4, stream);
            hipLaunchKernelGGL(k_members_check, dim3((n_members + 255) / 256), dim3(256), 0, stream, members, n_members, status, veto);
        }
#define RGX_COOP(PIECE_, WIN_) hipLaunchKernelGGL((k_inflate_coop<false, PIECE_, WIN_>), dim3(blocks), dim3(64), kInflateLdsBytes, stream, comp, members, n_members, arena, upos_bias, len_scratch, status, ignore_below, index_bias, bad, two, perm, veto, gate)
        if (piece) { if (win) RGX_COOP(true, 1); else RGX_COOP(true, 0); }
        else { if (win) RGX_COOP(false, 1); else RGX_COOP(false, 0); }
#undef RGX_COOP
        break;
    }
    default: {
        const bool lits4 = form == 5 || (plan & 2) != 0;
#define RGX_LANE(PIECE_, LITS_) hipLaunchKernelGGL((k_inflate<false, PIECE_, LITS_>), dim3(blocks), dim3(64), kInflateLdsBytes, stream, comp, members, n_members, arena, upos_bias, len_scratch, status, ignore_below, index_bias, bad)
        if (piece) { if (lits4) RGX_LANE(true, 4); else RGX_LANE(true, 1); }
        else { if (lits4) RGX_LANE(false, 4); else RGX_LANE(false, 1); }
#undef RGX_LANE
    }
    }
}
void launch_inflate_probe(const uint8_t *comp, const Member *members, uint32_t n_members, uint8_t *slots, uint32_t *len_scratch, uint32_t *sizes,
                          hipStream_t stream) {
    if (!n_members) return;
    inflate_attrs();
    const int form = inflate_form_env() ? inflate_form_env() : kDefaultLaneForm;
    const uint32_t blocks = (n_members + 63) / 64;
    if (form == 3) hipLaunchKernelGGL(k_inflate_ring<true>, dim3(blocks), dim3(64), kRingLdsBytes, stream, comp, members, n_members, slots, (uint64_t)0, len_scratch, sizes, 0u, 0u, (uint8_t *)nullptr);
    else if (form == 4) hipLaunchKernelGGL(k_inflate_coop<true>, dim3(blocks), dim3(64), kInflateLdsBytes, stream, comp, members, n_members, slots, (uint64_t)0, len_scratch, sizes, 0u, 0u, (uint8_t *)nullptr, 1u, (const uint32_t *)nullptr, (const uint32_t *)nullptr, InflateGate());
    else hipLaunchKernelGGL(k_inflate<true>, dim3(blocks), dim3(64), kInflateLdsBytes, stream, comp, members, n_members, slots, (uint64_t)0, len_scratch, sizes, 0u, 0u, (uint8_t *)nullptr);
}

__device__ __forceinline__ uint64_t walk_chain(const uint8_t *arena, uint64_t o, uint64_t seg_end, uint64_t lim, uint32_t &cnt, uint16_t *cp = nullptr,
                                               uint64_t seg_begin = 0, bool lite = false) {
    cnt = 0;
    while (o < seg_end) {
        if (o + 36 > lim) return kChainEnd;
        RecHead h;
        if (lite) {
            h.block_len = (int32_t)ld32(arena + o);
            if (h.block_len < 32) return kChainEnd;
        } else {
            rec_head(arena + o, h);
            if (!rec_sane(h)) return kChainEnd;
        }
        uint64_t nxt = o + 4 + (uint64_t)(uint32_t)h.block_len;
        if (nxt > lim) return kChainEnd;
        if (cp && (cnt & 7u) == 0) cp[cnt >> 3] = (uint16_t)(o - seg_begin);
        ++cnt;
        o = nxt;
    }
    return o;
}

__device__ __forceinline__ void seg_of(const SegGeom &g, uint32_t s, uint64_t &a, uint64_t &b, uint64_t &lim, bool &first) {
    if (!g.chunks) {
        a = g.pos0 + (uint64_t)s * g.seg_bytes; b = a + g.seg_bytes; lim = g.lim; first = s == 0;
        if (b > lim) b = lim;
        return;
    }
    uint32_t lo = 0, hi = g.n_chunks;
    while (hi - lo > 1) { const uint32_t mid = (lo + hi) >> 1; if (g.chunks[mid].seg_base <= s) lo = mid; else hi = mid; }
    const SegChunk c = g.chunks[lo];
    a = c.a + (uint64_t)(s - c.seg_base) * g.seg_bytes; b = a + g.seg_bytes; lim = c.dlim; first = s == c.seg_base;
    if (b > c.b) b = c.b;
}

__global__ void k_seg_walk(const uint8_t *__restrict__ arena, SegGeom g, uint32_t n_seg, int32_t n_ref,
                           uint64_t *seg_start, uint64_t *seg_exit, uint32_t *seg_cnt, uint16_t *seg_cp, uint32_t s_begin) {
    uint32_t s = s_begin + blockIdx.x * blockDim.x + threadIdx.x;
    if (s >= n_seg) return;
    uint16_t *cp = g.seg_bytes == kSegBytes ? seg_cp + (size_t)s * kSegCpSlots : nullptr;
    uint64_t a, b, lim; bool first;
    seg_of(g, s, a, b, lim, first);
    uint64_t o = a, ex = kChainEnd;
    uint32_t cnt = 0;
    if (!first) {
        o = kChainEnd;
        uint64_t c = a;
        for (;;) {
            uint64_t cand = kChainEnd;
            while (c < b) {
                const u32x4 v = ld128(arena + c);
                const uint32_t w[5] = {v[0], v[1], v[2], v[3], ld32(arena + c + 16)};
                uint32_t mask = 0;
#pragma unroll
                for (int i = 0; i < 16; ++i) {
                    const uint32_t bl = (i & 3) ? __builtin_amdgcn_alignbyte(w[(i >> 2) + 1], w[i >> 2], (uint32_t)(i & 3)) : w[i >> 2];
                    mask |= (bl - 32u <= (1u << 27) - 32u ? 1u : 0u) << i;
                }
                const uint64_t room = b - c;
                if (room < 16) mask &= (1u << (uint32_t)room) - 1u;
                bool found = false;
                while (mask) {
                    const uint32_t i = (uint32_t)__builtin_ctz(mask);
                    mask &= mask - 1;
                    const uint64_t q = c + i;
                    if (!rec_plausible(arena, q, lim, n_ref)) continue;
                    const uint64_t c2 = q + 4 + (uint64_t)ld32(arena + q);
                    if (c2 < lim) {
                        if (!rec_plausible(arena, c2, lim, n_ref)) continue;
                        const uint64_t c3 = c2 + 4 + (uint64_t)ld32(arena + c2);
                        if (c3 < lim && !rec_plausible(arena, c3, lim, n_ref)) continue;
                    }
                    cand = q; found = true; break;
                }
                if (found) break;
                c += 16;
            }
            if (cand == kChainEnd) break;
            ex = walk_chain(arena, cand, b, lim, cnt, cp, a, g.lite_walk != 0);
            if (ex != kChainEnd) { o = cand; break; }
            c = cand + 1;
        }
        if (o == kChainEnd) { ex = kChainUnknown; o = b; cnt = 0; }
    } else ex = walk_chain(arena, o, b, lim, cnt, cp, a, g.lite_walk != 0);
    seg_start[s] = o; seg_exit[s] = ex; seg_cnt[s] = cnt;
}

__device__ __forceinline__ bool seg_consistent(uint64_t b , uint64_t expect, uint64_t st, uint64_t ex, uint32_t cnt) {
    return expect >= b ? (st == b && ex == expect && cnt == 0) : st == expect;
}

__global__ void k_seg_verify(const uint8_t *__restrict__ arena, SegGeom g, uint32_t n_seg,
                             const uint64_t *__restrict__ st_in, const uint64_t *__restrict__ ex_in, const uint32_t *__restrict__ cnt_in,
                             uint64_t *st_out, uint64_t *ex_out, uint32_t *cnt_out, uint32_t *status, uint16_t *seg_cp) {
    uint32_t s = blockIdx.x * blockDim.x + threadIdx.x;
    if (s >= n_seg) return;
    uint64_t st = st_in[s], ex = ex_in[s];
    uint32_t cnt = cnt_in[s];
    uint64_t a, b, lim; bool first;
    seg_of(g, s, a, b, lim, first);
    if (ex == kChainEnd && (first || ex_in[s - 1] != kChainEnd)) atomicMin(status + 1, s);
    if (!first) {
        const uint64_t expect = ex_in[s - 1];
        if (expect == kChainUnknown) atomicMin(status, s);
        else if (!seg_consistent(b, expect, st, ex, cnt)) {
            atomicMin(status, s);
            const bool placeholder = ex == kChainUnknown;
            uint64_t a1, b1, lim1; bool first1;
            seg_of(g, s - 1, a1, b1, lim1, first1);
            const bool left_settled = first1 || (ex_in[s - 2] != kChainUnknown && seg_consistent(b1, ex_in[s - 2], st_in[s - 1], expect, cnt_in[s - 1]));
            if (placeholder || left_settled) {
                if (expect >= b) { st = b; ex = expect; cnt = 0; }
                else { st = expect; ex = walk_chain(arena, st, b, lim, cnt, g.seg_bytes == kSegBytes ? seg_cp + (size_t)s * kSegCpSlots : nullptr, a, g.lite_walk != 0); }
            }
        }
    }
    st_out[s] = st; ex_out[s] = ex; cnt_out[s] = cnt;
}

__global__ void k_seg_truncate(SegGeom g, uint32_t n_seg, uint32_t last, uint64_t *st, uint64_t *ex, uint32_t *cnt) {
    uint32_t s = blockIdx.x * blockDim.x + threadIdx.x;
    if (s >= n_seg || s <= last) return;
    uint64_t a, b, lim; bool first;
    seg_of(g, s, a, b, lim, first);
    st[s] = b; ex[s] = kChainEnd; cnt[s] = 0;
}

void launch_seg_walk(const uint8_t *arena, SegGeom g, uint32_t n_seg, int32_t n_ref, uint64_t *seg_start,
                     uint64_t *seg_exit, uint32_t *seg_cnt, uint16_t *seg_cp, hipStream_t stream, uint32_t s_begin) {
    if (n_seg <= s_begin) return;
    hipLaunchKernelGGL(k_seg_walk, dim3((n_seg - s_begin + 63) / 64), dim3(64), 0, stream, arena, g, n_seg, n_ref, seg_start, seg_exit, seg_cnt, seg_cp, s_begin);
}
void launch_seg_verify(const uint8_t *arena, SegGeom g, uint32_t n_seg, const uint64_t *seg_start_in,
                       const uint64_t *seg_exit_in, const uint32_t *seg_cnt_in, uint64_t *seg_start_out, uint64_t *seg_exit_out,
                       uint32_t *seg_cnt_out, uint32_t *status, uint16_t *seg_cp, hipStream_t stream) {
    if (!n_seg) return;
    hipLaunchKernelGGL(k_seg_verify, dim3((n_seg + 63) / 64), dim3(64), 0, stream, arena, g, n_seg, seg_start_in, seg_exit_in,
                       seg_cnt_in, seg_start_out, seg_exit_out, seg_cnt_out, status, seg_cp);
}
void launch_seg_truncate(SegGeom g, uint32_t n_seg, uint32_t last, uint64_t *seg_start, uint64_t *seg_exit, uint32_t *seg_cnt, hipStream_t stream) {
    if (!n_seg) return;
    hipLaunchKernelGGL(k_seg_truncate, dim3((n_seg + 255) / 256), dim3(256), 0, stream, g, n_seg, last, seg_start, seg_exit, seg_cnt);
}

constexpr uint32_t kSegTail = 1024;
constexpr uint32_t kSegMaxRecs = kSegBytes / 36 + 2;
template <bool STAGED>
__global__ __launch_bounds__(64) void k_decode_seg(const uint8_t *__restrict__ arena, SegGeom g, uint32_t n_seg,
                                                   const uint64_t *__restrict__ seg_start, const uint32_t *__restrict__ seg_base,
                                                   const uint32_t *__restrict__ seg_cnt, ExtractCfg cfg, ReadSoA soa, uint32_t *seg_iter,
                                                   uint32_t *seg_long, const uint16_t *__restrict__ seg_cp, uint32_t s_begin) {
    extern __shared__ __attribute__((aligned(16))) uint8_t s_buf[];
    __shared__ uint32_t s_off[kSegMaxRecs];
    const uint32_t s = s_begin + blockIdx.x, lane = threadIdx.x;
    const uint32_t cnt = seg_cnt[s];
    if (cnt == 0) { if (lane == 0) { seg_iter[s] = 0; seg_long[s] = 0; } return; }
    uint64_t a, seg_b, seg_lim; bool seg_first;
    seg_of(g, s, a, seg_b, seg_lim, seg_first);
    const uint64_t w0 = a & ~15ull;
    uint64_t w1 = a + kSegBytes + kSegTail;
    if (w1 > g.data_end) w1 = g.data_end;
    if constexpr (STAGED) {
        constexpr int kChunks = (kSegBytes + kSegTail + 16 + 1023) / 1024;
        u32x4 r[kChunks];
#pragma unroll
        for (int j = 0; j < kChunks; ++j) {
            const uint64_t o = w0 + (uint64_t)j * 1024 + (uint64_t)lane * 16;
            if (o < w1) r[j] = ld128(arena + o);
        }
#pragma unroll
        for (int j = 0; j < kChunks; ++j) {
            const uint64_t o = w0 + (uint64_t)j * 1024 + (uint64_t)lane * 16;
            if (o < w1) *(u32x4 *)(s_buf + (o - w0)) = r[j];
        }
    }
    __syncthreads();
    const uint32_t *s_w = (const uint32_t *)s_buf;
    auto lds32 = [&](uint32_t off) -> uint32_t {
        if constexpr (STAGED) return __builtin_amdgcn_alignbyte(s_w[(off >> 2) + 1], s_w[off >> 2], off & 3u);
        else return ld32(arena + w0 + off);
    };
    if (lane * 8 < cnt) {
        uint64_t o = a + seg_cp[(size_t)s * kSegCpSlots + lane];
        const uint32_t k_end = min(cnt, lane * 8 + 8);
        for (uint32_t k = lane * 8; k < k_end; ++k) {
            const uint32_t ro = (uint32_t)(o - w0);
            s_off[k] = ro;
            o += 4 + (uint64_t)((STAGED && o + 4 <= w1) ? lds32(ro) : ld32(arena + o));
        }
    }
    __syncthreads();
    const uint32_t base = seg_base[s];
    uint32_t n_iter = 0, n_long = 0;
    uint32_t first_stop = 0xffffffffu, last_in = 0;
    for (uint32_t k = lane; k < cnt; k += 64) {
        const uint32_t ro = s_off[k];
        const uint64_t o = w0 + ro;
        RecHead h;
        {
            const uint32_t sh = ro & 3u, wi = ro >> 2;
            uint32_t x[8];
            if constexpr (STAGED) {
                uint32_t d[9];
#pragma unroll
                for (int q = 0; q < 9; ++q) d[q] = s_w[wi + q];
#pragma unroll
                for (int q = 0; q < 8; ++q) x[q] = __builtin_amdgcn_alignbyte(d[q + 1], d[q], sh);
            } else {
                (void)sh; (void)wi;
#pragma unroll
                for (int q = 0; q < 8; ++q) x[q] = ld32(arena + o + 4 * q);
            }
            h.block_len = (int32_t)x[0]; h.tid = (int32_t)x[1]; h.pos = (int32_t)x[2];
            h.l_qname = x[3] & 0xff; h.n_cigar = x[4] & 0xffff; h.flag = x[4] >> 16;
            h.l_qseq = (int32_t)x[5]; h.mtid = (int32_t)x[6];
            h.aux_off = (int64_t)h.l_qname + 4 * (int64_t)h.n_cigar + (((int64_t)h.l_qseq + 1) >> 1) + h.l_qseq;
        }
        if (cfg.insane_out && !rec_sane(h)) { cfg.insane_out[0] = 1; h.n_cigar = 0; }
        const uint64_t rec_end = o + 4 + (uint64_t)(uint32_t)h.block_len;
        const bool in_win = STAGED && rec_end <= w1;
        const uint32_t cig_ro = ro + 36 + h.l_qname;
        const uint8_t *g_data = arena + o + 36;
        auto cigar_at = [&](uint32_t q) -> uint32_t { return in_win ? lds32(cig_ro + 4 * q) : ld32(g_data + h.l_qname + 4 * (size_t)q); };
        const uint32_t i = base + k;
        soa.tid[i] = h.tid; soa.pos[i] = h.pos;
        soa.flag_nc[i] = h.flag << 16 | h.n_cigar;
        soa.cig_off[i] = o + 36 + h.l_qname;
        if (soa.rec_off) soa.rec_off[i] = o;
        bool in_region = true;
        if (cfg.region_tid != -2) {
            in_region = h.tid == cfg.region_tid && h.pos < cfg.region_end;
            if (cfg.stop_out) {
                if (i >= cfg.stop_index) in_region = false;
                else if (!in_region) first_stop = min(first_stop, i);
            }
            if (in_region) {
                int32_t endpos = h.pos + 1;
                if (!(h.flag & 4) && h.n_cigar > 0) {
                    int32_t l = 0;
                    for (uint32_t q = 0; q < h.n_cigar; ++q) l += (int32_t)cig_ref_len(cigar_at(q));
                    endpos = h.pos + l;
                }
                in_region = endpos > cfg.region_beg;
            }
        }
        n_iter += in_region ? 1u : 0u;
        if (in_region) last_in = i + 1;
        uint32_t nev = 0;
        char strand = '?';
        uint8_t odd = 0;
        if (in_region && h.n_cigar > 1 && h.tid >= 0 && h.tid < cfg.n_ref) {
            if (cfg.bc0 && cfg.abort_out) {
                const int64_t l_data = (int64_t)h.block_len - 32;
                bool unknown = false;
                if (in_win) { const uint8_t *body = s_buf + ro + 36; (void)strand_from_tag(body + h.aux_off, body + l_data, cfg.bc0, cfg.bc1, &unknown); }
                else (void)strand_from_tag(g_data + h.aux_off, g_data + l_data, cfg.bc0, cfg.bc1, &unknown);
                if (unknown) atomicMin(cfg.abort_out, i);
            }
            bool has_n = false;
            for (uint32_t q = 0; q < h.n_cigar; ++q) {
                const uint32_t c = cigar_at(q);
                if (cig_is_N(c)) { const uint32_t len = c >> 4; nev += !(len < cfg.min_intron || len > cfg.max_intron); has_n = true; }
            }
            if (nev || (has_n && (cfg.abort_out || cfg.odd_count) && cfg.strandness == 0)) {
                if (cfg.strandness == 0) {
                    const int64_t l_data = (int64_t)h.block_len - 32;
                    bool unknown = false;
                    if (in_win) { const uint8_t *body = s_buf + ro + 36; strand = strand_from_tag(body + h.aux_off, body + l_data, cfg.tag0, cfg.tag1, &unknown); }
                    else strand = strand_from_tag(g_data + h.aux_off, g_data + l_data, cfg.tag0, cfg.tag1, &unknown);
                    if (unknown && cfg.abort_out) atomicMin(cfg.abort_out, i);
                    if (unknown && cfg.odd_count) { atomicAdd(cfg.odd_count, 1u); odd = 0x80; }
                } else strand = strand_from_flag(h.flag, cfg.strandness);
                if (nev) n_long += h.n_cigar > cfg.long_threshold ? 1u : 0u;
            }
        }
        soa.strand[i] = (uint8_t)strand | odd;
        soa.n_ev[i] = nev;
    }
    n_iter = wave_incl_scan(n_iter); n_long = wave_incl_scan(n_long);
    if (lane == 63) { seg_iter[s] = n_iter; seg_long[s] = n_long; }
    if (cfg.stop_out) {
#pragma unroll
        for (int d = 32; d > 0; d >>= 1) { first_stop = min(first_stop, (uint32_t)__shfl_xor((int)first_stop, d, 64)); last_in = max(last_in, (uint32_t)__shfl_xor((int)last_in, d, 64)); }
        if (lane == 0) {
            if (first_stop < *(volatile uint32_t *)&cfg.stop_out[0]) atomicMin(&cfg.stop_out[0], first_stop);
            if (last_in > *(volatile uint32_t *)&cfg.stop_out[1]) atomicMax(&cfg.stop_out[1], last_in);
        }
    }
}

__global__ __launch_bounds__(64) void k_decode_sparse(const uint8_t *__restrict__ arena, uint32_t n_seg, const uint64_t *__restrict__ seg_start,
                                                      const uint32_t *__restrict__ seg_base, const uint32_t *__restrict__ seg_cnt, ExtractCfg cfg, ReadSoA soa,
                                                      uint32_t *seg_iter, uint32_t *seg_long, uint32_t s_begin) {
    const uint32_t s = s_begin + blockIdx.x * 64 + threadIdx.x;
    uint32_t first_stop = 0xffffffffu, last_in = 0;
    if (s < n_seg) {
        const uint32_t cnt = seg_cnt[s];
        uint32_t n_iter = 0, n_long = 0;
        if (cnt) {
            uint64_t o = seg_start[s];
            const uint32_t base = seg_base[s];
            for (uint32_t k = 0; k < cnt; ++k) {
                RecHead h;
                rec_head(arena + o, h);
                if (cfg.insane_out && !rec_sane(h)) { cfg.insane_out[0] = 1; h.n_cigar = 0; }
                const uint8_t *g_data = arena + o + 36;
                auto cigar_at = [&](uint32_t q) -> uint32_t { return ld32(g_data + h.l_qname + 4 * (size_t)q); };
                const uint32_t i = base + k;
                soa.tid[i] = h.tid; soa.pos[i] = h.pos;
                soa.flag_nc[i] = h.flag << 16 | h.n_cigar;
                soa.cig_off[i] = o + 36 + h.l_qname;
                if (soa.rec_off) soa.rec_off[i] = o;
                bool in_region = true;
                if (cfg.region_tid != -2) {
                    in_region = h.tid == cfg.region_tid && h.pos < cfg.region_end;
                    if (cfg.stop_out) {
                        if (i >= cfg.stop_index) in_region = false;
                        else if (!in_region) first_stop = min(first_stop, i);
                    }
                    if (in_region) {
                        int32_t endpos = h.pos + 1;
                        if (!(h.flag & 4) && h.n_cigar > 0) {
                            int32_t l = 0;
                            for (uint32_t q = 0; q < h.n_cigar; ++q) l += (int32_t)cig_ref_len(cigar_at(q));
                            endpos = h.pos + l;
                        }
                        in_region = endpos > cfg.region_beg;
                    }
                }
                n_iter += in_region ? 1u : 0u;
                if (in_region) last_in = i + 1;
                uint32_t nev = 0;
                char strand = '?';
                uint8_t odd = 0;
                if (in_region && h.n_cigar > 1 && h.tid >= 0 && h.tid < cfg.n_ref) {
                    if (cfg.bc0 && cfg.abort_out) {
                        bool unknown = false;
                        (void)strand_from_tag(g_data + h.aux_off, g_data + ((int64_t)h.block_len - 32), cfg.bc0, cfg.bc1, &unknown);
                        if (unknown) atomicMin(cfg.abort_out, i);
                    }
                    bool has_n = false;
                    for (uint32_t q = 0; q < h.n_cigar; ++q) {
                        const uint32_t c = cigar_at(q);
                        if (cig_is_N(c)) { const uint32_t len = c >> 4; nev += !(len < cfg.min_intron || len > cfg.max_intron); has_n = true; }
                    }
                    if (nev || (has_n && (cfg.abort_out || cfg.odd_count) && cfg.strandness == 0)) {
                        if (cfg.strandness == 0) {
                            const int64_t l_data = (int64_t)h.block_len - 32;
                            bool unknown = false;
                            strand = strand_from_tag(g_data + h.aux_off, g_data + l_data, cfg.tag0, cfg.tag1, &unknown);
                            if (unknown && cfg.abort_out) atomicMin(cfg.abort_out, i);
                            if (unknown && cfg.odd_count) { atomicAdd(cfg.odd_count, 1u); odd = 0x80; }
                        } else strand = strand_from_flag(h.flag, cfg.strandness);
                        if (nev) n_long += h.n_cigar > cfg.long_threshold ? 1u : 0u;
                    }
                }
                soa.strand[i] = (uint8_t)strand | odd;
                soa.n_ev[i] = nev;
                o += 4 + (uint64_t)(uint32_t)h.block_len;
            }
        }
        seg_iter[s] = n_iter; seg_long[s] = n_long;
    }
    if (cfg.stop_out) {
#pragma unroll
        for (int d = 32; d > 0; d >>= 1) { first_stop = min(first_stop, (uint32_t)__shfl_xor((int)first_stop, d, 64)); last_in = max(last_in, (uint32_t)__shfl_xor((int)last_in, d, 64)); }
        if (threadIdx.x == 0) {
            if (first_stop < *(volatile uint32_t *)&cfg.stop_out[0]) atomicMin(&cfg.stop_out[0], first_stop);
            if (last_in > *(volatile uint32_t *)&cfg.stop_out[1]) atomicMax(&cfg.stop_out[1], last_in);
        }
    }
}

__global__ __launch_bounds__(64) void k_long_fill(uint32_t n_seg, const uint32_t *__restrict__ seg_base, const uint32_t *__restrict__ seg_cnt,
                                                  const uint32_t *__restrict__ seg_long_base, ExtractCfg cfg, ReadSoA soa, uint32_t *long_list) {
    const uint32_t s = blockIdx.x, lane = threadIdx.x;
    const uint32_t cnt = seg_cnt[s], base = seg_base[s];
    uint32_t out = seg_long_base[s];
    for (uint32_t k0 = 0; k0 < cnt; k0 += 64) {
        const uint32_t k = k0 + lane;
        bool is_long = false;
        if (k < cnt) is_long = soa.n_ev[base + k] != 0 && (soa.flag_nc[base + k] & 0xffff) > cfg.long_threshold;
        const uint64_t m = __ballot(is_long);
        if (is_long) long_list[out + (uint32_t)__popcll(m & lanemask_lt())] = base + k;
        out += (uint32_t)__popcll(m);
    }
}

const DecodeKnobs &decode_knobs() {
    static const DecodeKnobs k = [] {
        DecodeKnobs v;
        if (const char *e = getenv("REGTOOLS_AMD_DECODE")) {
            v.wave_form = !strncmp(e, "wave", 4);
            if (const char *c = strchr(e, ',')) v.seg_bytes = atoi(c + 1);
        }
        return v;
    }();
    return k;
}
void launch_decode_seg(const uint8_t *arena, SegGeom g, uint32_t n_seg, const uint64_t *seg_start, const uint32_t *seg_base,
                       const uint32_t *seg_cnt, ExtractCfg cfg, ReadSoA soa, uint32_t *seg_iter, uint32_t *seg_long, const uint16_t *seg_cp, bool staged, hipStream_t stream,
                       uint32_t s_begin) {
    if (n_seg <= s_begin) return;
    const uint32_t n = n_seg - s_begin;
    if (staged && g.seg_bytes == kSegBytes) hipLaunchKernelGGL(k_decode_seg<true>, dim3(n), dim3(64), kSegBytes + kSegTail + 48, stream, arena, g, n_seg, seg_start, seg_base, seg_cnt, cfg, soa, seg_iter, seg_long, seg_cp, s_begin);
    else {
        static const bool wave_form = decode_knobs().wave_form;
        if (wave_form && g.seg_bytes == kSegBytes) hipLaunchKernelGGL(k_decode_seg<false>, dim3(n), dim3(64), 0, stream, arena, g, n_seg, seg_start, seg_base, seg_cnt, cfg, soa, seg_iter, seg_long, seg_cp, s_begin);
        else hipLaunchKernelGGL(k_decode_sparse, dim3((n + 63) / 64), dim3(64), 0, stream, arena, n_seg, seg_start, seg_base, seg_cnt, cfg, soa, seg_iter, seg_long, s_begin);
    }
}
__global__ void k_collect_odd_aux(const uint8_t *__restrict__ arena, ReadSoA soa, uint32_t n_rec, uint32_t cap, uint32_t *count, int32_t *out) {
    const uint32_t i = blockIdx.x * blockDim.x + threadIdx.x;
    if (i >= n_rec || !(soa.strand[i] & 0x80u)) return;
    const uint32_t fnc = soa.flag_nc[i];
    const int32_t pos = soa.pos[i];
    const uint32_t k = atomicAdd(count, 1u);
    if (k < cap) { out[3 * (size_t)k] = soa.tid[i]; out[3 * (size_t)k + 1] = pos; out[3 * (size_t)k + 2] = rec_endpos(arena + soa.cig_off[i], fnc & 0xffffu, fnc >> 16, pos); }
}
void launch_collect_odd_aux(const uint8_t *arena, ReadSoA soa, uint32_t n_rec, uint32_t cap, uint32_t *count, int32_t *out, hipStream_t stream) {
    if (n_rec) hipLaunchKernelGGL(k_collect_odd_aux, dim3((n_rec + 255) / 256), dim3(256), 0, stream, arena, soa, n_rec, cap, count, out);
}
void launch_long_fill(uint32_t n_seg, const uint32_t *seg_base, const uint32_t *seg_cnt, const uint32_t *seg_long_base, ExtractCfg cfg, ReadSoA soa,
                      uint32_t *long_list, hipStream_t stream) {
    if (n_seg) hipLaunchKernelGGL(k_long_fill, dim3(n_seg), dim3(64), 0, stream, n_seg, seg_base, seg_cnt, seg_long_base, cfg, soa, long_list);
}


__device__ __forceinline__ void put_event(const EventSoA &ev, uint32_t slot, int32_t tid, uint32_t start, uint32_t end, uint32_t ts,
                                          uint32_t te, char strand, uint32_t rpos, uint32_t rend, uint32_t read) {
    if (ev.read) ev.read[slot] = read;
    ev.tid[slot] = (uint32_t)tid; ev.start[slot] = start;
    ev.ilen_cls[slot] = (end - start) << 2 | strand_class(strand);
    ev.ts[slot] = ts; ev.te[slot] = te; ev.strand[slot] = (uint8_t)strand;
    if (ev.rpos) { ev.rpos[slot] = rpos; ev.rend[slot] = rend; }
}

__global__ void k_emit_short(const uint8_t *__restrict__ arena, uint32_t n_rec, ExtractCfg cfg, ReadSoA soa,
                             const uint32_t *__restrict__ ev_base, EventSoA ev, uint32_t row_begin, const uint32_t *__restrict__ part_totals, uint32_t n_parts, uint32_t slot_cap) {
    uint32_t i = row_begin + blockIdx.x * blockDim.x + threadIdx.x;
    if (i >= n_rec) return;
    uint32_t nev = soa.n_ev[i];
    if (!nev) return;
    uint32_t fnc = soa.flag_nc[i], n_cigar = fnc & 0xffff;
    if (n_cigar > cfg.long_threshold) return;
    const uint8_t *cig = arena + soa.cig_off[i];
    int32_t tid = soa.tid[i];
    char strand = (char)soa.strand[i];
    uint32_t slot = ev_base[i];
    for (uint32_t k = 0; k < n_parts; ++k) slot += part_totals[k];
    const int32_t pos = soa.pos[i];
    const uint32_t rend = ev.rpos ? (uint32_t)rec_endpos(cig, n_cigar, fnc >> 16, pos) : 0u;
    char carried = 0;
    cigar_walk(pos, cig, n_cigar, [&](uint32_t s, uint32_t e, uint32_t ts, uint32_t te) {
        char st = strand;
        if (cfg.fa_data) {
            const FaContig fc = cfg.fa_tab[tid];
            if (!fc.present) { cfg.fa_missing[0] = 1u + (uint32_t)tid; }
            else { const char m = strand_from_motif(cfg.fa_data, fc, s, e, carried); if (m != '?') st = m; }
            carried = st;
        }
        if (intron_ok(s, e, cfg.min_intron, cfg.max_intron)) { if (slot < slot_cap) put_event(ev, slot, tid, s, e, ts, te, st, (uint32_t)pos, rend, i); ++slot; }
    });
}

__global__ __launch_bounds__(256) void k_emit_long(const uint8_t *__restrict__ arena, const uint32_t *__restrict__ long_list,
                                                   uint32_t n_long, ExtractCfg cfg, ReadSoA soa,
                                                   const uint32_t *__restrict__ ev_base, EventSoA ev) {
    __shared__ uint32_t s_ops[4][64];
    __shared__ uint32_t s_R[4][65];
    const uint32_t wave = threadIdx.x >> 6, lane = lane_id();
    const uint32_t stride = gridDim.x * 4;
    uint32_t w = blockIdx.x * 4 + wave;
    if (w >= n_long) return;
    uint32_t nx_i = long_list[w];
    uint32_t nn_i = w + stride < n_long ? long_list[w + stride] : 0u;
    uint32_t nx_fnc = soa.flag_nc[nx_i], nx_slot = ev_base[nx_i];
    uint64_t nx_cig = soa.cig_off[nx_i];
    int32_t nx_tid = soa.tid[nx_i], nx_pos = soa.pos[nx_i];
    uint8_t nx_strand = soa.strand[nx_i];
    for (; w < n_long; w += stride) {
        const uint32_t i = nx_i, fnc = nx_fnc;
        const uint32_t n_cigar = fnc & 0xffff;
        const uint8_t *cig = arena + nx_cig;
        const int32_t tid = nx_tid;
        const char strand = (char)nx_strand;
        uint32_t slot = nx_slot;
        const uint32_t rpos = (uint32_t)nx_pos;
        const uint32_t c_first = lane < n_cigar ? ld32(cig + 4 * (size_t)lane) : 0x5u ;
        if (w + stride < n_long) {
            nx_i = nn_i;
            nx_fnc = soa.flag_nc[nx_i]; nx_slot = ev_base[nx_i]; nx_cig = soa.cig_off[nx_i]; nx_tid = soa.tid[nx_i]; nx_pos = soa.pos[nx_i]; nx_strand = soa.strand[nx_i];
            if (w + 2 * stride < n_long) nn_i = long_list[w + 2 * stride];
        }
        uint32_t rend = 0;
        if (ev.rpos) {
            uint32_t span = 0;
            for (uint32_t t0 = lane; t0 < n_cigar; t0 += 64) span += cig_ref_len(ld32(cig + 4 * (size_t)t0));
            span = __shfl(wave_incl_scan(span), 63, 64);
            rend = ((fnc >> 16) & 4u) ? rpos + 1 : rpos + span;
        }
        uint32_t refpos = rpos;
        uint32_t ts_carry = refpos;
        bool pend = false; uint32_t p_start = 0, p_end = 0, p_ts = 0; char p_strand = strand;
        char carried = 0;
        for (uint32_t t0 = 0; t0 < n_cigar; t0 += 64) {
            const uint32_t k = t0 + lane;
            const uint32_t c = t0 == 0 ? c_first : k < n_cigar ? ld32(cig + 4 * (size_t)k) : 0x5u ;
            s_ops[wave][lane] = c;
            const uint32_t adv = cig_advances_junction_state(c) ? (c >> 4) : 0u;
            const uint32_t incl = wave_incl_scan(adv);
            const uint32_t R_before = refpos + incl - adv, R_after = refpos + incl;
            s_R[wave][lane] = R_before;
            if (lane == 63) s_R[wave][64] = R_after;
            const bool brk = k < n_cigar && cig_is_breaker(c);
            const bool isN = k < n_cigar && cig_is_N(c);
            const uint64_t B = __ballot(brk);
            __builtin_amdgcn_wave_barrier();
            if (pend && B) {
                const uint32_t nb = (uint32_t)__ffsll((unsigned long long)B) - 1;
                const uint32_t te = s_R[wave][nb];
                if (lane == 0 && intron_ok(p_start, p_end, cfg.min_intron, cfg.max_intron)) put_event(ev, slot, tid, p_start, p_end, p_ts, te, p_strand, rpos, rend, i);
                if (intron_ok(p_start, p_end, cfg.min_intron, cfg.max_intron)) ++slot;
                pend = false;
            }
            const uint64_t below = B & lanemask_lt();
            const uint64_t above = lane == 63 ? 0ull : (B >> (lane + 1)) << (lane + 1);
            const uint32_t ts = below ? s_R[wave][(63 - (uint32_t)__clzll((long long)below)) + 1] : ts_carry;
            const bool closed = above != 0;
            const uint32_t te = closed ? s_R[wave][(uint32_t)__ffsll((unsigned long long)above) - 1] : 0u;
            const bool ok = isN && intron_ok(R_before, R_after, cfg.min_intron, cfg.max_intron);
            char my_strand = strand;
            if (cfg.fa_data) {
                const FaContig fc = cfg.fa_tab[tid];
                char sA = strand, sB = strand;
                if (isN) {
                    if (!fc.present) cfg.fa_missing[0] = 1u + (uint32_t)tid;
                    else {
                        const char mA = strand_from_motif(cfg.fa_data, fc, R_before, R_after, 0), mB = strand_from_motif(cfg.fa_data, fc, R_before, R_after, '-');
                        if (mA != '?') sA = mA;
                        if (mB != '?') sB = mB;
                    }
                }
                uint64_t nm = __ballot(isN);
                while (nm) {
                    const uint32_t l = (uint32_t)__ffsll((unsigned long long)nm) - 1; nm &= nm - 1;
                    const char a = (char)__shfl((int)sA, l, 64), b = (char)__shfl((int)sB, l, 64);
                    const char s = carried == '-' ? b : a;
                    if (lane == l) my_strand = s;
                    carried = s;
                }
            }
            const uint64_t emit_mask = __ballot(ok && closed);
            if (ok && closed) put_event(ev, slot + (uint32_t)__popcll(emit_mask & lanemask_lt()), tid, R_before, R_after, ts, te, my_strand, rpos, rend, i);
            slot += (uint32_t)__popcll(emit_mask);
            if (B) {
                const uint32_t lastb = 63 - (uint32_t)__clzll((long long)B);
                const uint32_t lc = s_ops[wave][lastb];
                ts_carry = s_R[wave][lastb + 1];
                if (cig_is_N(lc)) {
                    pend = true;
                    p_start = s_R[wave][lastb]; p_end = s_R[wave][lastb + 1];
                    const uint64_t bl = B & ((1ull << lastb) - 1ull);
                    p_ts = __shfl(ts, lastb, 64);
                    p_strand = (char)__shfl((int)my_strand, lastb, 64);
                    (void)bl;
                }
            }
            refpos = __shfl(R_after, 63, 64);
            __builtin_amdgcn_wave_barrier();
        }
        if (pend && lane == 0 && intron_ok(p_start, p_end, cfg.min_intron, cfg.max_intron)) put_event(ev, slot, tid, p_start, p_end, p_ts, refpos, p_strand, rpos, rend, i);
    }
}

void launch_emit_short(const uint8_t *arena, uint32_t n_rec, ExtractCfg cfg, ReadSoA soa, const uint32_t *ev_base, EventSoA ev,
                       hipStream_t stream, uint32_t row_begin, const uint32_t *part_totals, uint32_t n_parts, uint32_t slot_cap) {
    if (n_rec <= row_begin) return;
    hipLaunchKernelGGL(k_emit_short, dim3((n_rec - row_begin + 255) / 256), dim3(256), 0, stream, arena, n_rec, cfg, soa, ev_base, ev, row_begin, part_totals, n_parts, slot_cap);
}
void launch_emit_long(const uint8_t *arena, const uint32_t *long_list, uint32_t n_long, ExtractCfg cfg,
                      ReadSoA soa, const uint32_t *ev_base, EventSoA ev, hipStream_t stream) {
    if (!n_long) return;
    uint32_t blocks = (n_long + 3) / 4;
    if (blocks > 256 * 8) blocks = 256 * 8;
    hipLaunchKernelGGL(k_emit_long, dim3(blocks), dim3(256), 0, stream, arena, long_list, n_long, cfg, soa, ev_base, ev);
}

constexpr uint32_t kScanTile = 4096;

__device__ __forceinline__ uint32_t block_excl_scan_256(uint32_t v, uint32_t *s_wave , uint32_t &block_total) {
    const uint32_t incl = wave_incl_scan(v);
    const uint32_t w = threadIdx.x >> 6;
    if (lane_id() == 63) s_wave[w] = incl;
    __syncthreads();
    uint32_t off = 0;
#pragma unroll
    for (uint32_t k = 0; k < 4; ++k) off += (k < w) ? s_wave[k] : 0u;
    block_total = s_wave[0] + s_wave[1] + s_wave[2] + s_wave[3];
    __syncthreads();
    return off + incl - v;
}

__global__ __launch_bounds__(256) void k_scan_reduce(const uint32_t *__restrict__ in, uint32_t n, uint32_t *tile_sum) {
    __shared__ uint32_t s_wave[4];
    const uint32_t base = blockIdx.x * kScanTile + threadIdx.x * 16;
    uint32_t sum = 0;
#pragma unroll
    for (uint32_t k = 0; k < 16; ++k) sum += (base + k < n) ? in[base + k] : 0u;
    uint32_t tot; block_excl_scan_256(sum, s_wave, tot);
    if (threadIdx.x == 0) tile_sum[blockIdx.x] = tot;
}

__global__ __launch_bounds__(256) void k_scan_tiles(uint32_t *tile_sum, uint32_t n_tiles, uint32_t *total) {
    __shared__ uint32_t s_wave[4];
    uint32_t carry = 0;
    for (uint32_t base = 0; base < n_tiles; base += 256) {
        const uint32_t i = base + threadIdx.x;
        const uint32_t v = i < n_tiles ? tile_sum[i] : 0u;
        uint32_t tot; const uint32_t ex = block_excl_scan_256(v, s_wave, tot);
        if (i < n_tiles) tile_sum[i] = carry + ex;
        carry += tot;
    }
    if (threadIdx.x == 0 && total) *total = carry;
}

__global__ __launch_bounds__(256) void k_scan_apply(const uint32_t *__restrict__ in, uint32_t *out, uint32_t n, const uint32_t *__restrict__ tile_sum) {
    __shared__ uint32_t s_wave[4];
    const uint32_t base = blockIdx.x * kScanTile + threadIdx.x * 16;
    uint32_t v[16], sum = 0;
#pragma unroll
    for (uint32_t k = 0; k < 16; ++k) { v[k] = (base + k < n) ? in[base + k] : 0u; sum += v[k]; }
    uint32_t tot; uint32_t run = block_excl_scan_256(sum, s_wave, tot) + tile_sum[blockIdx.x];
#pragma unroll
    for (uint32_t k = 0; k < 16; ++k) { if (base + k < n) out[base + k] = run; run += v[k]; }
}

size_t scan_tmp_words(uint32_t n) { return (size_t)(n + kScanTile - 1) / kScanTile + 1; }

void launch_scan_u32(const uint32_t *in, uint32_t *out, uint32_t n, uint32_t *total, uint32_t *tmp, hipStream_t stream) {
    if (!n) { if (total) (void)hipMemsetAsync(total, 0, 4, stream); return; }
    const uint32_t tiles = (n + kScanTile - 1) / kScanTile;
    hipLaunchKernelGGL(k_scan_reduce, dim3(tiles), dim3(256), 0, stream, in, n, tmp);
    hipLaunchKernelGGL(k_scan_tiles, dim3(1), dim3(256), 0, stream, tmp, tiles, total);
    hipLaunchKernelGGL(k_scan_apply, dim3(tiles), dim3(256), 0, stream, in, out, n, tmp);
}

constexpr uint32_t kRadixRowsLarge = 32, kRadixRowsSmall = 8, kRadixSmallMax = 2u << 20;
static inline uint32_t radix_rows(uint32_t n) {
    return n <= kRadixSmallMax ? kRadixRowsSmall : kRadixRowsLarge;
}

__device__ __forceinline__ uint32_t radix_digit(const uint32_t *__restrict__ word, const uint32_t *__restrict__ perm_in, uint32_t i,
                                                uint32_t shift, uint32_t mask, uint32_t &src) {
    src = perm_in ? perm_in[i] : i;
    return (word[src] >> shift) & mask;
}

__device__ __forceinline__ uint64_t match_digit(uint32_t d, bool valid) {
    uint64_t m = __ballot(valid);
#pragma unroll
    for (uint32_t b = 0; b < 8; ++b) {
        const uint64_t bal = __ballot((d >> b) & 1u);
        m &= ((d >> b) & 1u) ? bal : ~bal;
    }
    return m;
}

template <bool KEYED>
__global__ __launch_bounds__(64) void k_radix_hist(const uint32_t *__restrict__ word, uint32_t shift, uint32_t mask,
                                                   const uint32_t *__restrict__ perm_in, uint32_t n, uint32_t n_tiles, uint32_t *hist, uint32_t rows) {
    __shared__ uint32_t s_cnt[256];
    for (uint32_t k = threadIdx.x; k < 256; k += 64) s_cnt[k] = 0;
    __syncthreads();
    const uint32_t base = blockIdx.x * 64 * rows;
    for (uint32_t r = 0; r < rows; ++r) {
        const uint32_t i = base + r * 64 + threadIdx.x;
        if (i < n) { uint32_t src; atomicAdd(&s_cnt[KEYED ? ((word[i] >> shift) & mask) : radix_digit(word, perm_in, i, shift, mask, src)], 1u); }
    }
    __syncthreads();
    for (uint32_t k = threadIdx.x; k < 256; k += 64) hist[(size_t)k * n_tiles + blockIdx.x] = s_cnt[k];
}

template <bool KEYED>
__global__ __launch_bounds__(64) void k_radix_scatter(const uint32_t *__restrict__ word, uint32_t shift, uint32_t mask,
                                                      const uint32_t *__restrict__ perm_in, uint32_t *perm_out, uint32_t n,
                                                      uint32_t n_tiles, const uint32_t *__restrict__ hist_scan, uint32_t *key_out,
                                                      const uint32_t *__restrict__ digit_total, uint32_t rows) {
    __shared__ uint32_t s_base[256];
    {
        const uint32_t k0 = threadIdx.x * 4;
        const uint32_t t0 = digit_total[k0], t1 = digit_total[k0 + 1], t2 = digit_total[k0 + 2], t3 = digit_total[k0 + 3];
        const uint32_t incl = wave_incl_scan(t0 + t1 + t2 + t3);
        uint32_t run = incl - (t0 + t1 + t2 + t3);
        s_base[k0] = run + hist_scan[(size_t)k0 * n_tiles + blockIdx.x]; run += t0;
        s_base[k0 + 1] = run + hist_scan[(size_t)(k0 + 1) * n_tiles + blockIdx.x]; run += t1;
        s_base[k0 + 2] = run + hist_scan[(size_t)(k0 + 2) * n_tiles + blockIdx.x]; run += t2;
        s_base[k0 + 3] = run + hist_scan[(size_t)(k0 + 3) * n_tiles + blockIdx.x];
    }
    __syncthreads();
    const uint32_t base = blockIdx.x * 64 * rows;
    for (uint32_t r = 0; r < rows; ++r) {
        const uint32_t i = base + r * 64 + threadIdx.x;
        const bool valid = i < n;
        uint32_t src = 0, key = 0;
        uint32_t d = 0;
        if (KEYED) { if (valid) { key = word[i]; src = perm_in ? perm_in[i] : i; d = (key >> shift) & mask; } }
        else d = valid ? radix_digit(word, perm_in, i, shift, mask, src) : 0u;
        const uint64_t m = match_digit(d, valid);
        if (valid) {
            const uint32_t rank = (uint32_t)__popcll(m & lanemask_lt());
            const uint32_t leader = (uint32_t)__ffsll((unsigned long long)m) - 1;
            uint32_t b = 0;
// ... 429 lines not shown
```

regtools_amd/csrc/scalars.h:

```cpp
#pragma once
#include <stddef.h>
#include "kernels.h"
struct InflateStatus { uint32_t first_bad, code; };
struct Scalars {
    InflateStatus inflate;
    uint32_t spare2, n_rec;
    struct Counts {
        uint32_t n_events, n_long, n_unique, n_partial, n_iterated, spare9;
    } counts;
    struct Framing { uint32_t disagree, chain_end; } framing;
    InflateStatus hdr_inflate;
    uint32_t spare14[2], n_cand, n_members;
    uint32_t stop, spare19;
    uint64_t total_inflated;
    uint32_t spare22[2], q_index[3], spare27[5];
    uint64_t q_upos[3], spare38, q_coff[3];
    uint32_t spare46[14], variant_hits, junction_items, max_span, window_pairs;
    unsigned long long variant_visits, junction_visits;
    uint32_t assoc_pairs, fa_missing;
    uint32_t merge_unique, spare71;
    struct Barcodes { uint32_t not_string, hash_clash, n_pairs; } barcodes;
    uint32_t barcode_text_len;
    InflateStatus inflate_early; uint32_t spare78[2];
    struct Stop { uint32_t index, last_pass; } stop_rule;
    uint32_t insane, wait_timed_out;
    uint32_t part_events[rgx::kGateParts];
    uint64_t exit_staging, spare94;
    uint32_t abort_row;
    uint32_t odd_aux, spare98[2];
    InflateStatus trial_inflate; uint32_t spare102[26];
};
static_assert(sizeof(Scalars) == 512, "the scalar block is 512 bytes of HBM, inside the 4 KiB of pinned staging");
static_assert(offsetof(Scalars, inflate_early) - offsetof(Scalars, inflate) == rgx::kStatusEarly * 4, "k_inflate_* write status + kStatusEarly");
constexpr size_t kScalarsHeaderPart = offsetof(Scalars, n_cand), kScalarsQueryPart = offsetof(Scalars, variant_visits);
static_assert(kScalarsHeaderPart == 64 && kScalarsQueryPart == 256, "the front read-backs keep their sizes");

template <class T> inline hipError_t fetch_scalar(const Scalars *d_sc, Scalars *h_sc, T &host_member, hipStream_t st) {
    return hipMemcpyAsync(&host_member, (const char *)d_sc + ((const char *)&host_member - (const char *)h_sc), sizeof(T), hipMemcpyDeviceToHost, st);
}
```

Baseline: 2.121 billion alignments/s.

## Fuse segment framing walk and record decode into one kernel with fixed row slots

Adds a fused kernel that frames each segment (finds record starts in an LDS-staged window) and decodes the records in the same block. Rows go into fixed per-segment slots sized from the mean record length, which removes the separate walk kernel, the record-count scan and a host readback before decode. Padding rows are zeroed. If a segment overflows its slots, finds no record start, or the neighbour check disagrees, the code falls back to the old walk + decode path, which costs a redundant pass. Padded rows also add scan and emit work across all rows.

```diff
diff --git a/regtools_amd/csrc/api_internal.h b/regtools_amd/csrc/api_internal.h
--- a/regtools_amd/csrc/api_internal.h
+++ b/regtools_amd/csrc/api_internal.h
@@ -404,6 +404,50 @@
     uint32_t *seg_iter_e = nullptr, *seg_long_e = nullptr, *seg_long_base_e = nullptr;
     uint16_t *seg_cp = nullptr;
     int cur = 0;
+    int restart_device_resident() {
+        mark("inflate verdict: not clean, starting over device-resident");
+        if (gated) { c->gate_distrust = true; if (trace) fprintf(stderr,
+            "[rgx trace] arrival gate: verdict not clean, this context no longer uses it\n"); }
+        HIP_TRY(join_B());
+        HIP_TRY(complete_upload());
+        HIP_TRY(hipStreamSynchronize(copy_q));
+        HIP_TRY(hipStreamSynchronize(st));
+        const int rc2 = prepare_events(c, d_bam, nullptr, bam_len, bai, bai_len, p, want_read_span, P, err, errlen, nullptr, false, region_to_file_end);
+        P.t_begin = t_begin;
+        return rc2;
+    }
+    bool fused = false; uint32_t rows_per_seg = 0; uint32_t n_rows = 0;
+    const char *fused_refused = nullptr;
+    int frame_fused(uint32_t n_s, uint32_t from, bool &clean) {
+        launch_frame_decode_seg(arena, geom, n_s, cfg, soa, rows_per_seg, seg_start[cur], seg_exit[cur], seg_cnt[cur], seg_base, seg_iter_e, seg_long_e,
+                                &d_sc->fused_flags, st, from);
+        HIP_TRY(hipMemsetAsync(&d_sc->framing, 0xff, sizeof d_sc->framing, st));
+        launch_seg_verify(arena, geom, n_s, seg_start[cur], seg_exit[cur], seg_cnt[cur], seg_start[cur ^ 1], seg_exit[cur ^ 1], seg_cnt[cur ^ 1],
+                          &d_sc->framing.disagree, seg_cp, st);
+        cur ^= 1;
+        HIP_TRY(fetch(h_sc->framing));
+        HIP_TRY(fetch(h_sc->fused_flags));
+        HIP_TRY(hipMemcpyAsync(&h_sc->exit_staging, seg_exit[cur] + (n_s - 1), 8, hipMemcpyDeviceToHost, st));
+        if (spec) {
+            HIP_TRY(fetch(h_sc->inflate));
+            HIP_TRY(fetch(h_sc->inflate_early));
+        }
+        HIP_TRY(hipStreamSynchronize(st));
+        if (spec && (h_sc->inflate.first_bad != 0xffffffffu || h_sc->inflate_early.first_bad != 0xffffffffu)) return restart_device_resident();
+        ++P.framing_sweeps;
+        const Scalars::Framing &fr = h_sc->framing;
+        fused_refused = (h_sc->fused_flags & kFusedOverflow) ? "a segment starts more records than it has rows" :
+                        (h_sc->fused_flags & kFusedPlaceholder) ? "a segment found no record start" :
+                        fr.chain_end != 0xffffffffu ? "the record chain ends" : fr.disagree != 0xffffffffu ? "a guess disagrees with its left neighbour" : nullptr;
+        clean = !fused_refused;
+        return -1;
+    }
+    hipError_t fused_fall_back() {
+        if (trace) fprintf(stderr, "[rgx trace] framing: fallback to walk + decode: %s\n", fused_refused ? fused_refused : "?");
+        fused = false; n_rows = 0;
+        if (cfg.abort_out) return hipMemsetAsync(&d_sc->abort_row, 0xff, 4, st);
+        return hipSuccess;
+    }
     int frame(uint32_t n_s, uint32_t walk_from, bool &ended) {
         DevBuf &b_tmp = c->buf(Buf::tmp);
         launch_seg_walk(arena, geom, n_s, n_ref, seg_start[cur], seg_exit[cur], seg_cnt[cur], seg_cp, st, walk_from);
@@ -420,18 +464,8 @@
                 HIP_TRY(fetch(h_sc->inflate_early));
             }
             HIP_TRY(hipStreamSynchronize(st));
-            if (spec && iter == 0 && (h_sc->inflate.first_bad != 0xffffffffu || h_sc->inflate_early.first_bad != 0xffffffffu)) {
-                mark("inflate verdict: not clean, starting over device-resident");
-                if (gated) { c->gate_distrust = true; if (trace) fprintf(stderr,
-                    "[rgx trace] arrival gate: verdict not clean, this context no longer uses it\n"); }
-                HIP_TRY(join_B());
-                HIP_TRY(complete_upload());
-                HIP_TRY(hipStreamSynchronize(copy_q));
-                HIP_TRY(hipStreamSynchronize(st));
-                const int rc2 = prepare_events(c, d_bam, nullptr, bam_len, bai, bai_len, p, want_read_span, P, err, errlen, nullptr, false, region_to_file_end);
-                P.t_begin = t_begin;
-                return rc2;
-            }
+            if (spec && iter == 0 && (h_sc->inflate.first_bad != 0xffffffffu || h_sc->inflate_early.first_bad != 0xffffffffu))
+                return restart_device_resident();
             ++P.framing_sweeps;
             const Scalars::Framing &fr = h_sc->framing;
             if (fr.chain_end != 0xffffffffu) ended = true;
diff --git a/regtools_amd/csrc/api_records.cpp b/regtools_amd/csrc/api_records.cpp
--- a/regtools_amd/csrc/api_records.cpp
+++ b/regtools_amd/csrc/api_records.cpp
@@ -229,7 +229,8 @@
         n_seg = lastc.seg_base + (uint32_t)((lastc.b - lastc.a + seg_bytes - 1) / seg_bytes);
         geom.data_end = total;
     }
-    n_rec = 0;
+    n_rec = 0; n_rows = 0;
+    fused = false; rows_per_seg = 0; fused_refused = nullptr;
     DevBuf &b_seg = c->buf(Buf::seg), &b_tmp = c->buf(Buf::tmp);
     HIP_TRY(hipEventRecord(c->ev[2], st));
     sA = 0;
@@ -253,6 +254,28 @@
         const bool env_early_emit = true;
         const bool small_ok = overlap_knobs().early_small;
         uint32_t waves_done = 0;
+        const char *why_walk = framing_knobs().force_walk ? "forced (REGTOOLS_AMD_FRAMING)" : seg_bytes != kSegBytes ? "long segments" :
+            (geom.chunks || !whole) ? "a region query" : (p->n_shards > 1 || cut_hi != UINT64_MAX) ? "a shard" : c->walk_strict ? "the strict walk" :
+            p->barcodes ? "barcodes" : want_read_span ? "read spans wanted" : (empty_stream || lim != total) ? "the stream ends early" :
+            !mean_rec ? "record size unknown" : mean_rec > kSparseRecordBytes ? "long records" : nullptr;
+        if (!why_walk) {
+            rows_per_seg = fused_rows_per_seg(mean_rec);
+            if ((uint64_t)n_seg * rows_per_seg >= 0xffffffffull) why_walk = "too many rows";
+        }
+        if (!why_walk) {
+            fused = true; n_rows = n_seg * rows_per_seg;
+            { const int rc = soa_layout(n_rows); if (rc != kGoOn) return rc; }
+            cfg.insane_out = nullptr;
+            if (lite_walk) { cfg.insane_out = &d_sc->insane; HIP_TRY(hipMemsetAsync(&d_sc->insane, 0, 4, st)); h_sc->insane = 0; }
+            HIP_TRY(hipMemsetAsync(&d_sc->fused_flags, 0, 4, st));
+        } else if (trace) fprintf(stderr, "[rgx trace] framing: walk + decode (%s)\n", why_walk);
+        const uint32_t sweeps_call = P.framing_sweeps;
+        auto drop_fused = [&](const char *why) -> hipError_t {
+            if (!fused) return hipSuccess;
+            if (!fused_refused) fused_refused = why;
+            P.framing_sweeps = sweeps_call;
+            return fused_fall_back();
+        };
         for (size_t j = 0; early && j < early_parts.size(); ++j) {
             const EarlyPart &ep = early_parts[j];
             if (ep.upos <= pos0 + 2 * (uint64_t)kBgzfMaxBlock) continue;
@@ -265,14 +288,16 @@
             }
             HIP_TRY(fetch(h_sc->wait_timed_out));
             if (trace) fprintf(stderr, "[rgx trace] early tail: part %zu: members < %u, segments [%u, %u) of %u\n", j, ep.members, sA, sJ, n_seg);
-            bool ended_J = false;
+            bool ended_J = false, clean_J = true;
             const uint32_t sweeps0 = P.framing_sweeps;
-            const int rcJ = frame(sJ, sA, ended_J);
+            const int rcJ = fused ? frame_fused(sJ, sA, clean_J) : frame(sJ, sA, ended_J);
             if (rcJ != -1) return rcJ;
-            const uint32_t n_rec_J = h_sc->n_rec;
+            const uint32_t n_rec_J = fused ? sJ * rows_per_seg : h_sc->n_rec;
             uint64_t exit_J = 0;
-            HIP_TRY(hipMemcpyAsync(&h_sc->exit_staging, seg_exit[cur] + (sJ - 1), 8, hipMemcpyDeviceToHost, st));
-            HIP_TRY(hipStreamSynchronize(st));
+            if (!fused) {
+                HIP_TRY(hipMemcpyAsync(&h_sc->exit_staging, seg_exit[cur] + (sJ - 1), 8, hipMemcpyDeviceToHost, st));
+                HIP_TRY(hipStreamSynchronize(st));
+            }
             exit_J = h_sc->exit_staging;
             const bool reaches_J = exit_J > ep.upos;
             if (reaches_J && trace) fprintf(stderr,
@@ -283,14 +308,17 @@
             const uint64_t span_J = (uint64_t)sJ * seg_bytes;
             if (h_sc->wait_timed_out) { c->early_distrust = true; if (trace) fprintf(stderr,
                 "[rgx trace] early tail: a wait for a part's waves timed out, this context no longer uses it\n"); }
-            if (h_sc->wait_timed_out || ended_J || slow_J || reaches_J || !n_rec_J || span_J / n_rec_J > kSparseRecordBytes ||
-                (sA && n_rec_J > soa_cap)) { early = false; sA = 0; emit_parts_ok = false; emit_parts = 0; emit_rows = 0; break; }
-            if (!sA) {
+            if (h_sc->wait_timed_out || ended_J || slow_J || reaches_J || !clean_J || !n_rec_J || (!fused && span_J / n_rec_J > kSparseRecordBytes) ||
+                (sA && n_rec_J > soa_cap)) {
+                HIP_TRY(drop_fused("the early tail was given up"));
+                early = false; sA = 0; emit_parts_ok = false; emit_parts = 0; emit_rows = 0; break;
+            }
+            if (!sA && !fused) {
                 { const int rc = soa_layout((size_t)((double)n_rec_J * ((double)n_seg / sJ) * 1.125) + 65536); if (rc != kGoOn) return rc; }
                 cfg.insane_out = nullptr;
                 if (lite_walk) { cfg.insane_out = &d_sc->insane; HIP_TRY(hipMemsetAsync(&d_sc->insane, 0, 4, st)); h_sc->insane = 0; }
             }
-            launch_decode_seg(arena, geom, sJ, seg_start[cur], seg_base, seg_cnt[cur], cfg, soa, seg_iter_e, seg_long_e, seg_cp, true, st, sA);
+            if (!fused) launch_decode_seg(arena, geom, sJ, seg_start[cur], seg_base, seg_cnt[cur], cfg, soa, seg_iter_e, seg_long_e, seg_cp, true, st, sA);
             if (!sA) {
                 DevBuf &b_ev0 = c->buf(Buf::events);
                 ev_lay = b_ev0.cap > 256 ? (b_ev0.cap - 256) / kEventRowBytes : 0;
@@ -308,9 +336,18 @@
             mark("early tail: part framed and decoded");
         }
         HIP_TRY(join_B());
-        const int rcF = frame(n_seg, sA, chain_ended);
-        if (rcF != -1) return rcF;
-        n_rec = h_sc->n_rec;
+        if (fused) {
+            bool clean = true;
+            const int rcF = frame_fused(n_seg, sA, clean);
+            if (rcF != -1) return rcF;
+            if (!clean) { HIP_TRY(drop_fused("?")); sA = 0; emit_parts_ok = false; emit_parts = 0; emit_rows = 0; }
+            else if (trace) fprintf(stderr, "[rgx trace] framing: fused, %u segments of %u rows\n", n_seg, rows_per_seg);
+        }
+        if (!fused) {
+            const int rcF = frame(n_seg, sA, chain_ended);
+            if (rcF != -1) return rcF;
+            n_rec = h_sc->n_rec; n_rows = n_rec;
+        }
     } else HIP_TRY(join_B());
     if (spec && !n_seg) {
         HIP_TRY(fetch(h_sc->inflate));
@@ -342,32 +379,35 @@
     DevBuf &b_tmp = c->buf(Buf::tmp);
     n_events = 0; n_long = 0;
     n_iterated = 0;
-    if (n_rec) {
-        const size_t R = n_rec;
+    if (n_rows) {
+        const size_t R = n_rows;
         uint32_t s_from = sA;
-        if (sA && (R > soa_cap || chain_ended)) s_from = 0;
-        if (!s_from) { const int rc = soa_layout(R); if (rc != kGoOn) return rc; emit_parts_ok = false; }
-        HIP_TRY(b_tmp.ensure(scan_tmp_words(n_rec) * 4 + 64));
-        uint32_t *seg_iter = sA ? seg_iter_e : seg_cnt[cur ^ 1], *seg_long = sA ? seg_long_e : (uint32_t *)seg_start[cur ^ 1], *seg_long_base = sA ?
+        if (!fused) {
+            if (sA && (R > soa_cap || chain_ended)) s_from = 0;
+            if (!s_from) { const int rc = soa_layout(R); if (rc != kGoOn) return rc; emit_parts_ok = false; }
+        }
+        HIP_TRY(b_tmp.ensure(scan_tmp_words(n_rows) * 4 + 64));
+        const bool own = sA || fused;
+        uint32_t *seg_iter = own ? seg_iter_e : seg_cnt[cur ^ 1], *seg_long = own ? seg_long_e : (uint32_t *)seg_start[cur ^ 1], *seg_long_base = own ?
             seg_long_base_e : (uint32_t *)seg_exit[cur ^ 1];
         if (geom.chunks) {
             cfg.stop_out = &d_sc->stop_rule.index; cfg.stop_index = 0xffffffffu;
             HIP_TRY(hipMemsetAsync(&d_sc->stop_rule.index, 0xff, 4, st));
             HIP_TRY(hipMemsetAsync(&d_sc->stop_rule.last_pass, 0, 4, st));
         }
-        if (!s_from) {
+        if (!s_from && !fused) {
             cfg.insane_out = nullptr;
             if (lite_walk) { cfg.insane_out = &d_sc->insane; HIP_TRY(hipMemsetAsync(&d_sc->insane, 0, 4, st)); h_sc->insane = 0; }
         }
         for (int pass = 0; pass < 2; ++pass) {
-            launch_decode_seg(arena, geom, n_seg, seg_start[cur], seg_base, seg_cnt[cur], cfg, soa, seg_iter, seg_long, seg_cp,
-                              span / n_rec <= kSparseRecordBytes, st, s_from);
+            if (!fused) launch_decode_seg(arena, geom, n_seg, seg_start[cur], seg_base, seg_cnt[cur], cfg, soa, seg_iter, seg_long, seg_cp,
+                                          span / n_rec <= kSparseRecordBytes, st, s_from);
             if (emit_parts_ok && s_from) {
-                launch_scan_u32(soa.n_ev + emit_rows, ev_base + emit_rows, n_rec - emit_rows, d_sc->part_events + emit_parts, b_tmp.as<uint32_t>(), st);
-                launch_emit_short(arena, n_rec, cfg, soa, ev_base, ev_e, st, emit_rows, d_sc->part_events, emit_parts,
+                launch_scan_u32(soa.n_ev + emit_rows, ev_base + emit_rows, n_rows - emit_rows, d_sc->part_events + emit_parts, b_tmp.as<uint32_t>(), st);
+                launch_emit_short(arena, n_rows, cfg, soa, ev_base, ev_e, st, emit_rows, d_sc->part_events, emit_parts,
                     (uint32_t)std::min<size_t>(ev_lay, 0xffffffffu));
                 HIP_TRY(fetch(h_sc->part_events));
-            } else launch_scan_u32(soa.n_ev, ev_base, n_rec, &d_sc->counts.n_events, b_tmp.as<uint32_t>(), st);
+            } else launch_scan_u32(soa.n_ev, ev_base, n_rows, &d_sc->counts.n_events, b_tmp.as<uint32_t>(), st);
             launch_scan_u32(seg_iter, seg_iter, n_seg, &d_sc->counts.n_iterated, b_tmp.as<uint32_t>(), st);
             launch_scan_u32(seg_long, seg_long_base, n_seg, &d_sc->counts.n_long, b_tmp.as<uint32_t>(), st);
             HIP_TRY(fetch(h_sc->counts));
@@ -399,19 +439,20 @@
             for (uint32_t k = 0; k <= emit_parts && k < kGateParts; ++k) tot += h_sc->part_events[k];
             if (tot > ev_lay || tot > 0xffffffffull || n_long) {
                 emit_parts_ok = false;
-                launch_scan_u32(soa.n_ev, ev_base, n_rec, &d_sc->counts.n_events, b_tmp.as<uint32_t>(), st);
+                launch_scan_u32(soa.n_ev, ev_base, n_rows, &d_sc->counts.n_events, b_tmp.as<uint32_t>(), st);
                 HIP_TRY(fetch(h_sc->counts.n_events));
                 HIP_TRY(hipStreamSynchronize(st));
                 n_events = h_sc->counts.n_events;
             } else n_events = (uint32_t)tot;
         }
         n_iterated = h_sc->counts.n_iterated;
+        if (fused) n_rec = h_sc->counts.n_iterated;
         if (cfg.odd_count && h_sc->odd_aux) {
             const uint32_t cap = h_sc->odd_aux;
             DevBuf &b_odd = c->buf(Buf::odd_aux);
             HIP_TRY(b_odd.ensure((size_t)cap * 12 + 16));
             HIP_TRY(hipMemsetAsync(&d_sc->odd_aux, 0, 4, st));
-            launch_collect_odd_aux(arena, soa, n_rec, cap, &d_sc->odd_aux, b_odd.as<int32_t>(), st);
+            launch_collect_odd_aux(arena, soa, n_rows, cap, &d_sc->odd_aux, b_odd.as<int32_t>(), st);
             HIP_TRY(fetch(h_sc->odd_aux));
             HIP_TRY(hipStreamSynchronize(st));
             const uint32_t n_odd = std::min(h_sc->odd_aux, cap);
@@ -433,11 +474,11 @@
     EventSoA ev; memset(&ev, 0, sizeof ev);
     if (n_events) {
         const size_t E = n_events;
-        if (emit_parts_ok && n_rec) ev = ev_e;
+        if (emit_parts_ok && n_rows) ev = ev_e;
         else {
             HIP_TRY(b_ev.ensure(E * kEventRowBytes + 256));
             Carve w(b_ev); ev = ev_layout(w, E); CARVE_TRY(w, "events");
-            launch_emit_short(arena, n_rec, cfg, soa, ev_base, ev, st);
+            launch_emit_short(arena, n_rows, cfg, soa, ev_base, ev, st);
             launch_emit_long(arena, long_list, n_long, cfg, soa, ev_base, ev, st);
         }
         if (cfg.fa_data) {
diff --git a/regtools_amd/csrc/bam_core.h b/regtools_amd/csrc/bam_core.h
--- a/regtools_amd/csrc/bam_core.h
+++ b/regtools_amd/csrc/bam_core.h
@@ -28,17 +28,89 @@
     return h.aux_off <= l_data;
 }
 
-RGX_HD bool rec_plausible(const uint8_t *arena, uint64_t o, uint64_t lim, int32_t n_ref) {
+template <class Rd32>
+RGX_HD void rec_head_rd(Rd32 &&rd32, uint64_t o, RecHead &h) {
+    h.block_len = (int32_t)rd32(o);
+    h.tid = (int32_t)rd32(o + 4); h.pos = (int32_t)rd32(o + 8);
+    uint32_t x2 = rd32(o + 12), x3 = rd32(o + 16);
+    h.l_qname = x2 & 0xff; h.n_cigar = x3 & 0xffff; h.flag = x3 >> 16;
+    h.l_qseq = (int32_t)rd32(o + 20);
+    h.mtid = (int32_t)rd32(o + 24);
+    h.aux_off = (int64_t)h.l_qname + 4 * (int64_t)h.n_cigar + (((int64_t)h.l_qseq + 1) >> 1) + h.l_qseq;
+}
+
+template <class Rd32, class Rd8>
+RGX_HD bool rec_plausible_rd(Rd32 &&rd32, Rd8 &&rd8, uint64_t o, uint64_t lim, int32_t n_ref) {
     if (o + 36 > lim) return false;
-    RecHead h; rec_head(arena + o, h);
+    if (rd32(o) - 32u > (1u << 27) - 32u) return false;
+    RecHead h; rec_head_rd(rd32, o, h);
     if (!rec_sane(h)) return false;
-    if (h.block_len > (1 << 27)) return false;
     if (h.tid < -1 || h.tid >= n_ref || h.mtid < -1 || h.mtid >= n_ref) return false;
     if (h.pos < -1 || h.pos > (1 << 29)) return false;
     uint64_t q_end = o + 36 + h.l_qname - 1;
-    if (q_end < lim && arena[q_end] != 0) return false;
+    if (q_end < lim && rd8(q_end) != 0) return false;
     return true;
 }
+RGX_HD bool rec_plausible(const uint8_t *arena, uint64_t o, uint64_t lim, int32_t n_ref) {
+    return rec_plausible_rd([&](uint64_t q) { return ld32(arena + q); }, [&](uint64_t q) { return arena[q]; }, o, lim, n_ref);
+}
+
+constexpr uint64_t kChainEnd = ~0ull;
+constexpr uint64_t kChainUnknown = ~0ull - 1;
+
+template <class Rd32, class Rd8>
+RGX_HD bool start_plausible(Rd32 &&rd32, Rd8 &&rd8, uint64_t c, uint64_t lim, int32_t n_ref) {
+    if (!rec_plausible_rd(rd32, rd8, c, lim, n_ref)) return false;
+    const uint64_t c2 = c + 4 + (uint64_t)rd32(c);
+    if (c2 < lim) {
+        if (!rec_plausible_rd(rd32, rd8, c2, lim, n_ref)) return false;
+        const uint64_t c3 = c2 + 4 + (uint64_t)rd32(c2);
+        if (c3 < lim && !rec_plausible_rd(rd32, rd8, c3, lim, n_ref)) return false;
+    }
+    return true;
+}
+
+template <class Rd32, class Put>
+RGX_HD uint64_t walk_window(Rd32 &&rd32, Put &&put, uint64_t o, uint64_t seg_end, uint64_t lim, bool lite, uint32_t &cnt) {
+    cnt = 0;
+    while (o < seg_end) {
+        if (o + 36 > lim) return kChainEnd;
+        RecHead h;
+        if (lite) {
+            h.block_len = (int32_t)rd32(o);
+            if (h.block_len < 32) return kChainEnd;
+        } else {
+            rec_head_rd(rd32, o, h);
+            if (!rec_sane(h)) return kChainEnd;
+        }
+        const uint64_t nxt = o + 4 + (uint64_t)(uint32_t)h.block_len;
+        if (nxt > lim) return kChainEnd;
+        put(cnt, o);
+        ++cnt;
+        o = nxt;
+    }
+    return o;
+}
+
+struct WindowFrame { uint64_t start, exit; uint32_t cnt; };
+template <class Rd32, class Rd8, class FirstHit, class Put>
+RGX_HD WindowFrame frame_window(Rd32 &&rd32, Rd8 &&rd8, FirstHit &&first_hit, Put &&put, uint64_t a, uint64_t b, uint64_t lim, bool first, bool lite,
+                                int32_t n_ref) {
+    WindowFrame f;
+    if (first) { f.start = a; f.exit = walk_window(rd32, put, a, b, lim, lite, f.cnt); return f; }
+    uint64_t from = a;
+    for (;;) {
+        const uint64_t cand = first_hit(from, b, [&](uint64_t c) { return start_plausible(rd32, rd8, c, lim, n_ref); });
+        if (cand == kChainEnd) break;
+        f.start = cand; f.exit = walk_window(rd32, put, cand, b, lim, lite, f.cnt);
+        if (f.exit != kChainEnd) return f;
+        from = cand + 1;
+    }
+    f.start = b; f.exit = kChainUnknown; f.cnt = 0;
+    return f;
+}
+constexpr uint32_t kFusedOverflow = 1u, kFusedPlaceholder = 2u;
+RGX_HD uint32_t fused_verdict(const WindowFrame &f, uint32_t K) { return f.cnt > K ? kFusedOverflow : f.exit == kChainUnknown ? kFusedPlaceholder : 0u; }
 
 RGX_HD char strand_from_flag(uint32_t flag, int strandness) {
     int rev = (flag >> 4) & 1, mrev = (flag >> 5) & 1, r1 = (flag >> 6) & 1, r2 = (flag >> 7) & 1;
diff --git a/regtools_amd/csrc/kernels.h b/regtools_amd/csrc/kernels.h
--- a/regtools_amd/csrc/kernels.h
+++ b/regtools_amd/csrc/kernels.h
@@ -9,8 +9,6 @@
 constexpr uint32_t kSegBytes = 16384;
 constexpr uint32_t kSparseRecordBytes = 2048;
 constexpr uint32_t kSegCpSlots = 64;
-constexpr uint64_t kChainEnd = ~0ull;
-constexpr uint64_t kChainUnknown = ~0ull - 1;
 
 size_t inflate_scratch_bytes(uint32_t n_members);
 hipError_t pending_launch_error();
@@ -112,6 +110,17 @@
                        const uint32_t *seg_cnt, ExtractCfg cfg, ReadSoA soa, uint32_t *seg_iter, uint32_t *seg_long, const uint16_t *seg_cp,
                        bool staged , hipStream_t stream,
                        uint32_t s_begin = 0 );
+constexpr uint32_t kSegMaxRecs = kSegBytes / 36 + 2;
+inline uint32_t fused_rows_per_seg(uint32_t mean_rec) {
+    const uint32_t k = kSegBytes / (mean_rec ? mean_rec : 1u);
+    const uint32_t K = k + k / 4 + 8;
+    return K < kSegMaxRecs ? K : kSegMaxRecs;
+}
+struct FramingKnobs { bool force_walk = false; };
+const FramingKnobs &framing_knobs();
+void launch_frame_decode_seg(const uint8_t *arena, SegGeom g, uint32_t n_seg, ExtractCfg cfg, ReadSoA soa, uint32_t rows_per_seg, uint64_t *seg_start,
+                             uint64_t *seg_exit, uint32_t *seg_cnt, uint32_t *seg_base, uint32_t *seg_iter, uint32_t *seg_long, uint32_t *flags,
+                             hipStream_t stream, uint32_t s_begin = 0);
 void launch_long_fill(uint32_t n_seg, const uint32_t *seg_base, const uint32_t *seg_cnt, const uint32_t *seg_long_base, ExtractCfg cfg, ReadSoA soa,
                       uint32_t *long_list, hipStream_t stream);
 
diff --git a/regtools_amd/csrc/kernels.hip b/regtools_amd/csrc/kernels.hip
--- a/regtools_amd/csrc/kernels.hip
+++ b/regtools_amd/csrc/kernels.hip
@@ -651,53 +651,41 @@
 }
 
 constexpr uint32_t kSegTail = 1024;
-constexpr uint32_t kSegMaxRecs = kSegBytes / 36 + 2;
+constexpr uint32_t kSegLdsBytes = kSegBytes + kSegTail + 48;
+
+__device__ __forceinline__ void seg_window(const SegGeom &g, uint64_t a, uint64_t &w0, uint64_t &w1) {
+    w0 = a & ~15ull;
+    w1 = a + kSegBytes + kSegTail;
+    if (w1 > g.data_end) w1 = g.data_end;
+}
+__device__ __forceinline__ void stage_window(const uint8_t *__restrict__ arena, uint8_t *s_buf, uint64_t w0, uint64_t w1, uint32_t lane) {
+    constexpr int kChunks = (kSegBytes + kSegTail + 16 + 1023) / 1024;
+    u32x4 r[kChunks];
+#pragma unroll
+    for (int j = 0; j < kChunks; ++j) {
+        const uint64_t o = w0 + (uint64_t)j * 1024 + (uint64_t)lane * 16;
+        if (o < w1) r[j] = ld128(arena + o);
+    }
+#pragma unroll
+    for (int j = 0; j < kChunks; ++j) {
+        const uint64_t o = w0 + (uint64_t)j * 1024 + (uint64_t)lane * 16;
+        if (o < w1) *(u32x4 *)(s_buf + (o - w0)) = r[j];
+    }
+}
+__device__ __forceinline__ uint32_t lds32_at(const uint8_t *s_buf, uint32_t off) {
+    const uint32_t *s_w = (const uint32_t *)s_buf;
+    return __builtin_amdgcn_alignbyte(s_w[(off >> 2) + 1], s_w[off >> 2], off & 3u);
+}
+
 template <bool STAGED>
-__global__ __launch_bounds__(64) void k_decode_seg(const uint8_t *__restrict__ arena, SegGeom g, uint32_t n_seg,
-                                                   const uint64_t *__restrict__ seg_start, const uint32_t *__restrict__ seg_base,
-                                                   const uint32_t *__restrict__ seg_cnt, ExtractCfg cfg, ReadSoA soa, uint32_t *seg_iter,
-                                                   uint32_t *seg_long, const uint16_t *__restrict__ seg_cp, uint32_t s_begin) {
-    extern __shared__ __attribute__((aligned(16))) uint8_t s_buf[];
-    __shared__ uint32_t s_off[kSegMaxRecs];
-    const uint32_t s = s_begin + blockIdx.x, lane = threadIdx.x;
-    const uint32_t cnt = seg_cnt[s];
-    if (cnt == 0) { if (lane == 0) { seg_iter[s] = 0; seg_long[s] = 0; } return; }
-    uint64_t a, seg_b, seg_lim; bool seg_first;
-    seg_of(g, s, a, seg_b, seg_lim, seg_first);
-    const uint64_t w0 = a & ~15ull;
-    uint64_t w1 = a + kSegBytes + kSegTail;
-    if (w1 > g.data_end) w1 = g.data_end;
-    if constexpr (STAGED) {
-        constexpr int kChunks = (kSegBytes + kSegTail + 16 + 1023) / 1024;
-        u32x4 r[kChunks];
-#pragma unroll
-        for (int j = 0; j < kChunks; ++j) {
-            const uint64_t o = w0 + (uint64_t)j * 1024 + (uint64_t)lane * 16;
-            if (o < w1) r[j] = ld128(arena + o);
-        }
-#pragma unroll
-        for (int j = 0; j < kChunks; ++j) {
-            const uint64_t o = w0 + (uint64_t)j * 1024 + (uint64_t)lane * 16;
-            if (o < w1) *(u32x4 *)(s_buf + (o - w0)) = r[j];
-        }
-    }
-    __syncthreads();
+__device__ __forceinline__ void decode_rows(const uint8_t *__restrict__ arena, const uint8_t *s_buf, const uint32_t *s_off, uint64_t w0, uint64_t w1,
+                                            uint32_t s, uint32_t cnt, uint32_t base, const ExtractCfg &cfg, const ReadSoA &soa, uint32_t *seg_iter,
+                                            uint32_t *seg_long, uint32_t lane) {
     const uint32_t *s_w = (const uint32_t *)s_buf;
     auto lds32 = [&](uint32_t off) -> uint32_t {
-        if constexpr (STAGED) return __builtin_amdgcn_alignbyte(s_w[(off >> 2) + 1], s_w[off >> 2], off & 3u);
+        if constexpr (STAGED) return lds32_at(s_buf, off);
         else return ld32(arena + w0 + off);
     };
-    if (lane * 8 < cnt) {
-        uint64_t o = a + seg_cp[(size_t)s * kSegCpSlots + lane];
-        const uint32_t k_end = min(cnt, lane * 8 + 8);
-        for (uint32_t k = lane * 8; k < k_end; ++k) {
-            const uint32_t ro = (uint32_t)(o - w0);
-            s_off[k] = ro;
-            o += 4 + (uint64_t)((STAGED && o + 4 <= w1) ? lds32(ro) : ld32(arena + o));
-        }
-    }
-    __syncthreads();
-    const uint32_t base = seg_base[s];
     uint32_t n_iter = 0, n_long = 0;
     uint32_t first_stop = 0xffffffffu, last_in = 0;
     for (uint32_t k = lane; k < cnt; k += 64) {
@@ -794,6 +782,71 @@
             if (last_in > *(volatile uint32_t *)&cfg.stop_out[1]) atomicMax(&cfg.stop_out[1], last_in);
         }
     }
+}
+
+template <bool STAGED>
+__global__ __launch_bounds__(64) void k_decode_seg(const uint8_t *__restrict__ arena, SegGeom g, uint32_t n_seg,
+                                                   const uint64_t *__restrict__ seg_start, const uint32_t *__restrict__ seg_base,
+                                                   const uint32_t *__restrict__ seg_cnt, ExtractCfg cfg, ReadSoA soa, uint32_t *seg_iter,
+                                                   uint32_t *seg_long, const uint16_t *__restrict__ seg_cp, uint32_t s_begin) {
+    extern __shared__ __attribute__((aligned(16))) uint8_t s_buf[];
+    __shared__ uint32_t s_off[kSegMaxRecs];
+    const uint32_t s = s_begin + blockIdx.x, lane = threadIdx.x;
+    const uint32_t cnt = seg_cnt[s];
+    if (cnt == 0) { if (lane == 0) { seg_iter[s] = 0; seg_long[s] = 0; } return; }
+    uint64_t a, seg_b, seg_lim; bool seg_first;
+    seg_of(g, s, a, seg_b, seg_lim, seg_first);
+    uint64_t w0, w1;
+    seg_window(g, a, w0, w1);
+    if constexpr (STAGED) stage_window(arena, s_buf, w0, w1, lane);
+    __syncthreads();
+    if (lane * 8 < cnt) {
+        uint64_t o = a + seg_cp[(size_t)s * kSegCpSlots + lane];
+        const uint32_t k_end = min(cnt, lane * 8 + 8);
+        for (uint32_t k = lane * 8; k < k_end; ++k) {
+            const uint32_t ro = (uint32_t)(o - w0);
+            s_off[k] = ro;
+            o += 4 + (uint64_t)((STAGED && o + 4 <= w1) ? lds32_at(s_buf, ro) : ld32(arena + o));
+        }
+    }
+    __syncthreads();
+    decode_rows<STAGED>(arena, s_buf, s_off, w0, w1, s, cnt, seg_base[s], cfg, soa, seg_iter, seg_long, lane);
+}
+
+__global__ __launch_bounds__(64) void k_frame_decode_seg(const uint8_t *__restrict__ arena, SegGeom g, uint32_t n_seg, ExtractCfg cfg, ReadSoA soa,
+                                                         uint32_t K, uint64_t *seg_start, uint64_t *seg_exit, uint32_t *seg_cnt, uint32_t *seg_base,
+                                                         uint32_t *seg_iter, uint32_t *seg_long, uint32_t *flags, uint32_t s_begin) {
+    extern __shared__ __attribute__((aligned(16))) uint8_t s_buf[];
+    __shared__ uint32_t s_off[kSegMaxRecs];
+    const uint32_t s = s_begin + blockIdx.x, lane = threadIdx.x;
+    uint64_t a, seg_b, seg_lim; bool seg_first;
+    seg_of(g, s, a, seg_b, seg_lim, seg_first);
+    uint64_t w0, w1;
+    seg_window(g, a, w0, w1);
+    stage_window(arena, s_buf, w0, w1, lane);
+    __syncthreads();
+    auto rd32 = [&](uint64_t o) -> uint32_t { return o + 4 <= w1 ? lds32_at(s_buf, (uint32_t)(o - w0)) : ld32(arena + o); };
+    auto rd8 = [&](uint64_t o) -> uint8_t { return o < w1 ? s_buf[o - w0] : arena[o]; };
+    auto first_hit = [&](uint64_t from, uint64_t b, auto &&pred) -> uint64_t {
+        for (uint64_t cb = from; cb < b; cb += 64) {
+            const uint64_t c = cb + lane;
+            const uint64_t m = __ballot(c < b && pred(c));
+            if (m) return cb + (uint64_t)(__ffsll((unsigned long long)m) - 1);
+        }
+        return kChainEnd;
+    };
+    auto put = [&](uint32_t k, uint64_t o) { if (lane == 0 && k < kSegMaxRecs) s_off[k] = (uint32_t)(o - w0); };
+    const WindowFrame f = frame_window(rd32, rd8, first_hit, put, a, seg_b, seg_lim, seg_first, g.lite_walk != 0, cfg.n_ref);
+    const uint32_t verdict = fused_verdict(f, K);
+    const uint32_t base = s * K;
+    if (lane == 0) {
+        seg_start[s] = f.start; seg_exit[s] = f.exit; seg_cnt[s] = f.cnt; seg_base[s] = base;
+        if (verdict) atomicOr(flags, verdict);
+    }
+    if (verdict) { if (lane == 0) { seg_iter[s] = 0; seg_long[s] = 0; } return; }
+    __syncthreads();
+    for (uint32_t k = f.cnt + lane; k < K; k += 64) soa.n_ev[base + k] = 0;
+    decode_rows<true>(arena, s_buf, s_off, w0, w1, s, f.cnt, base, cfg, soa, seg_iter, seg_long, lane);
 }
 
 __global__ __launch_bounds__(64) void k_decode_sparse(const uint8_t *__restrict__ arena, uint32_t n_seg, const uint64_t *__restrict__ seg_start,
@@ -910,12 +963,27 @@
                        uint32_t s_begin) {
     if (n_seg <= s_begin) return;
     const uint32_t n = n_seg - s_begin;
-    if (staged && g.seg_bytes == kSegBytes) hipLaunchKernelGGL(k_decode_seg<true>, dim3(n), dim3(64), kSegBytes + kSegTail + 48, stream, arena, g, n_seg, seg_start, seg_base, seg_cnt, cfg, soa, seg_iter, seg_long, seg_cp, s_begin);
+    if (staged && g.seg_bytes == kSegBytes) hipLaunchKernelGGL(k_decode_seg<true>, dim3(n), dim3(64), kSegLdsBytes, stream, arena, g, n_seg, seg_start, seg_base, seg_cnt, cfg, soa, seg_iter, seg_long, seg_cp, s_begin);
     else {
         static const bool wave_form = decode_knobs().wave_form;
         if (wave_form && g.seg_bytes == kSegBytes) hipLaunchKernelGGL(k_decode_seg<false>, dim3(n), dim3(64), 0, stream, arena, g, n_seg, seg_start, seg_base, seg_cnt, cfg, soa, seg_iter, seg_long, seg_cp, s_begin);
         else hipLaunchKernelGGL(k_decode_sparse, dim3((n + 63) / 64), dim3(64), 0, stream, arena, n_seg, seg_start, seg_base, seg_cnt, cfg, soa, seg_iter, seg_long, s_begin);
     }
+}
+const FramingKnobs &framing_knobs() {
+    static const FramingKnobs k = [] {
+        FramingKnobs v;
+        if (const char *e = getenv("REGTOOLS_AMD_FRAMING")) v.force_walk = !strncmp(e, "walk", 4);
+        return v;
+    }();
+    return k;
+}
+void launch_frame_decode_seg(const uint8_t *arena, SegGeom g, uint32_t n_seg, ExtractCfg cfg, ReadSoA soa, uint32_t rows_per_seg, uint64_t *seg_start,
+                             uint64_t *seg_exit, uint32_t *seg_cnt, uint32_t *seg_base, uint32_t *seg_iter, uint32_t *seg_long, uint32_t *flags,
+                             hipStream_t stream, uint32_t s_begin) {
+    if (n_seg <= s_begin) return;
+    hipLaunchKernelGGL(k_frame_decode_seg, dim3(n_seg - s_begin), dim3(64), kSegLdsBytes, stream, arena, g, n_seg, cfg, soa, rows_per_seg, seg_start, seg_exit,
+                       seg_cnt, seg_base, seg_iter, seg_long, flags, s_begin);
 }
 __global__ void k_collect_odd_aux(const uint8_t *__restrict__ arena, ReadSoA soa, uint32_t n_rec, uint32_t cap, uint32_t *count, int32_t *out) {
     const uint32_t i = blockIdx.x * blockDim.x + threadIdx.x;
diff --git a/regtools_amd/csrc/scalars.h b/regtools_amd/csrc/scalars.h
--- a/regtools_amd/csrc/scalars.h
+++ b/regtools_amd/csrc/scalars.h
@@ -4,7 +4,7 @@
 struct InflateStatus { uint32_t first_bad, code; };
 struct Scalars {
     InflateStatus inflate;
-    uint32_t spare2, n_rec;
+    uint32_t fused_flags, n_rec;
     struct Counts {
         uint32_t n_events, n_long, n_unique, n_partial, n_iterated, spare9;
     } counts;
```

Result: slower. 1.850 billion alignments/s (-12.8%).
